# EnricoMiccoli/nodal

Measured on AMD Instinct MI355X. Metric: circuits_per_sec, higher is better.
Workload: dtype f64; 1 GPU; cfg3: grid(1000) 1e6 nodes, sparse CSR path; n=999999, nnz=4995995, parallelism=one GPU

## Files before the change

### nodal_amd/csrc/sagg.hip

```cpp
#include <hip/hip_ext.h>

#include <atomic>
#include <type_traits>

#include "group.h"

int grounded_flags(nodal_ctx *h, uint8_t *flags_dev);

namespace {

using grp::TB;
constexpr int PW = 4;
constexpr int ACAP = 64;
constexpr int RCAP = 96;
constexpr int RCAP_SMALL = 512;
constexpr int RCAP_SMALL_ROWS = 16384;
inline int rcap_for(int64_t nc) { return nc <= RCAP_SMALL_ROWS ? RCAP_SMALL : RCAP; }
constexpr int W0_MAX = 32;
constexpr int COARSEST = 64;
constexpr int MAX_LEVELS = 12;
constexpr int MIS_ROUNDS = 6;
constexpr int TAIL_MAX_N = 1024;
constexpr int TAIL_LEVELS = 6;
constexpr int TAIL_LDS_BUDGET = 150 * 1024;
constexpr int APAD = 32;
constexpr int DOT_BLOCKS = 1024;
#ifndef NODAL_SA_OMEGA
#define NODAL_SA_OMEGA 0.85
#endif
constexpr double OMEGA = NODAL_SA_OMEGA;
constexpr double OMEGA_P = 0.70;
constexpr double OMEGA_P_COARSE = 0.85;
using cyc_t = nodal_cyc_t;

inline unsigned grid_for(int64_t n, unsigned cap = 8192) {
    int64_t g = (n + TB - 1) / TB;
    if (g < 1) g = 1;
    if (g >= 64) g = (g + 7) & ~(int64_t)7;
    return (unsigned)(g > cap ? cap : g);
}
inline int64_t pad64(int64_t n) { return (n + 63) & ~(int64_t)63; }

__device__ __forceinline__ unsigned xcd_block() {
    const unsigned g = gridDim.x, b = blockIdx.x;
    return (g & 7u) ? b : (b & 7u) * (g >> 3) + (b >> 3);
}


struct Ell {
    int64_t n = 0, ld = 0;
    int32_t width = 0;
    const int32_t *col = nullptr;
    const int16_t *dcol = nullptr;
    const double *val = nullptr;
    const float *valf = nullptr;
    const int32_t *len = nullptr;
};

enum { ST_MAXLEN = 0, ST_GRADED = 1, ST_BADDIAG = 2, ST_OVERFLOW = 3, ST_NNZ = 4, ST_UNASSIGNED = 5,
       ST_MAXR = 6, ST_NC = 7 ,
       ST_FARCOL = 8 , ST_COUNT = 9 };

struct SLevel {
    int64_t n = 0, ld = 0, nc = 0;
    int32_t width = 0;
    int32_t maxlen = 0;
    int32_t wfix = 0;
    int64_t nnz = 0;
    DevBuf acol, aval, alen, dinv;
    DevBuf adcol;
    bool d16 = false;
    DevBuf agg, pcol, pval;
    DevBuf rcol, rval, rlen;
    int64_t rld = 0;
    DevBuf vec, part, gflag;
    DevBuf avalf, pvalf, rvalf;
    Ell A() const {
        Ell e;
        e.n = n; e.ld = ld; e.width = width;
        e.col = acol.as<int32_t>(); e.val = aval.as<double>(); e.len = alen.as<int32_t>();
        e.valf = avalf.as<float>();
        e.dcol = d16 ? adcol.as<int16_t>() : nullptr;
        return e;
    }
    template <typename T = double> T *v(int which) const { return reinterpret_cast<T *>(vec.as<double>() + (int64_t)which * ld); }
};
enum { V_X = 0, V_R = 1, V_XP = 2, V_RC = 3, V_C1 = 4, V_C2 = 5, V_V1 = 6, V_V2 = 7, V_R2 = 8, V_X1 = 9, V_T = 10,
       V_COUNT = 11 };

struct TailLevelDesc {
    int n, nc, ld, rld, width, nq, lpr;
    const int32_t *acol, *pcol, *rcol, *rlen, *alen;
    const double *aval, *dinv, *pval, *rval;
    int o_aval, o_acol, o_dinv, o_pval, o_pcol, o_rval, o_rcol, o_B, o_X, o_Y, o_R;
};
struct TailDesc {
    int nlev;
    TailLevelDesc lv[TAIL_LEVELS];
    const double *inv;
    int nu;
    int image_bytes;
    int lds_bytes;
    int skip;
    int slots;
    long long *stamps;
};

struct SHierarchy {
    std::vector<SLevel *> pool;
    int nlev = 0;
    int tail = -1;
    bool ready = false;
    bool kcycle = true;
    bool kfrozen = false;
    int kslot = -1, kcount = 0, ksamples = 0;
    int klevels = 1;
    int nu[3] = {2, 1, 2};
    bool dense_coarsest = true;
    DevBuf tail_stamps, tail_image, apcol, apval, aplen, bstat;
    DevBuf mvec;
    hipEvent_t ev_copy = nullptr;
    hipStream_t aux = nullptr;
    hipEvent_t ev_fork = nullptr, ev_join = nullptr, ev_flags = nullptr;
    bool aux_pending = false;
    bool aux_tried = false;
    bool want_flags = false;
    int flags_levels = 0;
    DevBuf stats, coarse_inv, mis_t, mis_m, mis_flag, mis_id, agg1, keys, rstart, cursor, lists;
    TailDesc td;
    uint64_t *host_stats = nullptr;
    bool sym_valid = false;
    uint64_t sym_epoch = 0;
    int64_t sym_n = 0, sym_nnz = 0;
    bool sym_general = false, sym_check = false;
    int32_t sym_floating = 0;
    hipGraph_t it_graph = nullptr;
    hipGraphExec_t it_exec = nullptr;
    uint64_t it_key = 0;
    bool refreshed = false;
    int last_iters = 0;
    int hint_iters = 0;
    int64_t hint_n = 0, hint_nnz = 0;
    int mblock_iters = 0;
    int64_t mblock_n = 0;
    unsigned long long sym_stats[MAX_LEVELS * ST_COUNT] = {0};
    SLevel *level(int l) {
        while ((int)pool.size() <= l) pool.push_back(new SLevel());
        return pool[l];
    }
    void drop_graph() {
        if (it_exec) (void)hipGraphExecDestroy(it_exec);
        if (it_graph) (void)hipGraphDestroy(it_graph);
        it_exec = nullptr;
        it_graph = nullptr;
        it_key = 0;
    }
    ~SHierarchy() {
        drop_graph();
        if (ev_copy) (void)hipEventDestroy(ev_copy);
        if (ev_fork) (void)hipEventDestroy(ev_fork);
        if (ev_join) (void)hipEventDestroy(ev_join);
        if (ev_flags) (void)hipEventDestroy(ev_flags);
        if (aux) (void)hipStreamDestroy(aux);
        for (SLevel *l : pool) {
            DevBuf *b[] = {&l->acol, &l->aval, &l->alen, &l->dinv, &l->agg, &l->pcol, &l->pval, &l->rcol,
                           &l->rval, &l->rlen, &l->vec, &l->part, &l->gflag, &l->avalf, &l->pvalf, &l->rvalf, &l->adcol};
            for (DevBuf *x : b) x->release();
            delete l;
        }
        tail_image.release();
        mvec.release();
        tail_stamps.release();
        bstat.release();
        apcol.release();
        apval.release();
        aplen.release();
        DevBuf *b[] = {&stats, &coarse_inv, &mis_t, &mis_m, &mis_flag, &mis_id, &agg1, &keys, &rstart, &cursor, &lists};
        for (DevBuf *x : b) x->release();
        if (host_stats) (void)hipHostFree(host_stats);
    }
};


constexpr int BSTAT_MAX = 65536;
__global__ __launch_bounds__(1024) void reduce_bstat(int nblocks, const uint32_t *__restrict__ bstat,
                                                     unsigned long long *__restrict__ stats, int slot_max,
                                                     int slot_sum) {
    __shared__ unsigned int s_max;
    __shared__ unsigned long long s_sum;
    if (threadIdx.x == 0) { s_max = 0; s_sum = 0; }
    __syncthreads();
    unsigned int m = 0;
    unsigned long long t = 0;
    for (int i = threadIdx.x; i < nblocks; i += 1024) {
        m = max(m, bstat[i]);
        t += bstat[BSTAT_MAX + i];
    }
    atomicMax(&s_max, m);
    atomicAdd(&s_sum, t);
    __syncthreads();
    if (threadIdx.x == 0) {
        if (slot_max >= 0) stats[slot_max] = s_max;
        if (slot_sum >= 0) stats[slot_sum] = s_sum;
    }
}

__global__ __launch_bounds__(TB) void row_stats(int64_t n, const int32_t *__restrict__ indptr,
                                                const int32_t *__restrict__ indices,
                                                const double *__restrict__ data, double share, double spread,
                                                bool general, unsigned long long *__restrict__ stats,
                                                uint32_t *__restrict__ bstat) {
    int32_t mlen = 0;
    uint32_t graded = 0, bad = 0, far = 0;
    for (int64_t i = (int64_t)xcd_block() * TB + threadIdx.x; i < n; i += (int64_t)gridDim.x * TB) {
        const int32_t e0 = indptr[i], e1 = indptr[i + 1];
        mlen = max(mlen, e1 - e0);
        double d = 0.0, mx = 0.0, mn = 1e300;
        for (int32_t e = e0; e < e1; ++e) {
            const double v = data[e];
            const int64_t dc = (int64_t)indices[e] - i;
            if (dc > 32767 || dc < -32767) far = 1;
            if (indices[e] == (int32_t)i) d = v;
            else if (v != 0.0) {
                mx = fmax(mx, fabs(v));
                mn = fmin(mn, fabs(v));
                if (v > 0.0 && !general) bad = 1;
            }
        }
        if (!(d > 0.0)) bad = 1;
        graded += (d > 0.0 && (mx > share * d || mx > spread * mn)) ? 1u : 0u;
    }
    __shared__ unsigned int s_len, s_graded, s_bad;
    if (threadIdx.x == 0) s_len = s_graded = s_bad = 0;
    __syncthreads();
    atomicMax(&s_len, (unsigned)mlen);
    if (graded) atomicAdd(&s_graded, graded);
    if (bad) atomicOr(&s_bad, 1u);
    if (far) atomicOr(&s_bad, 2u);
    __syncthreads();
    if (threadIdx.x == 0) {
        bstat[blockIdx.x] = s_len;
        bstat[BSTAT_MAX + blockIdx.x] = s_graded;
        if (s_bad & 1u) atomicOr(&stats[ST_BADDIAG], 1ull);
        if (s_bad & 2u) stats[ST_FARCOL] = 1ull;
    }
}

__global__ __launch_bounds__(TB) void csr_to_ell(int64_t n, int64_t ld, const int32_t *__restrict__ indptr,
                                                 const int32_t *__restrict__ indices,
                                                 const double *__restrict__ data, int32_t *__restrict__ col,
                                                 double *__restrict__ val, float *__restrict__ valf,
                                                 int32_t *__restrict__ len, double *__restrict__ dinv, int32_t wpad,
                                                 int16_t *__restrict__ dcol) {
    for (int64_t i = (int64_t)xcd_block() * TB + threadIdx.x; i < n; i += (int64_t)gridDim.x * TB) {
        const int32_t e0 = indptr[i], e1 = indptr[i + 1];
        double d = 1.0;
        for (int32_t e = e0; e < e1; ++e) {
            const int32_t c = indices[e];
            const double v = data[e];
            col[(int64_t)(e - e0) * ld + i] = c;
            if (dcol) dcol[(int64_t)(e - e0) * ld + i] = (int16_t)(c - (int32_t)i);
            val[(int64_t)(e - e0) * ld + i] = v;
            valf[(int64_t)(e - e0) * ld + i] = (float)v;
            if (c == (int32_t)i) d = v;
        }
        for (int32_t s = e1 - e0; s < wpad; ++s) {
            col[(int64_t)s * ld + i] = (int32_t)i;
            if (dcol) dcol[(int64_t)s * ld + i] = 0;
            val[(int64_t)s * ld + i] = 0.0;
            valf[(int64_t)s * ld + i] = 0.0f;
        }
        len[i] = e1 - e0;
        dinv[i] = 1.0 / d;
    }
}


__device__ __forceinline__ uint32_t hash30(uint32_t x) {
    x ^= x >> 16;
    x *= 0x7feb352du;
    x ^= x >> 15;
    x *= 0x846ca68bu;
    x ^= x >> 16;
    return x & 0x3fffffffu;
}

__global__ __launch_bounds__(TB) void mis_init(int64_t n, uint32_t *__restrict__ T) {
    for (int64_t i = (int64_t)xcd_block() * TB + threadIdx.x; i < n; i += (int64_t)gridDim.x * TB)
        T[i] = (1u << 30) | hash30((uint32_t)i);
}

template <int NB>
__device__ __forceinline__ uint32_t nbr_max_batch(const Ell &A, const uint32_t *__restrict__ v, int64_t i, int32_t l, int32_t s0,
                                                  uint32_t best) {
    int32_t c[NB];
#pragma unroll
    for (int u = 0; u < NB; ++u) c[u] = A.col[(int64_t)(s0 + u < l ? s0 + u : 0) * A.ld + i];
    uint32_t t[NB];
#pragma unroll
    for (int u = 0; u < NB; ++u) t[u] = v[c[u]];
#pragma unroll
    for (int u = 0; u < NB; ++u) best = t[u] > best ? t[u] : best;
    return best;
}
__device__ __forceinline__ uint32_t nbr_max(const Ell &A, const uint32_t *__restrict__ v, int64_t i, int32_t l, uint32_t best) {
    if (l <= 5) return nbr_max_batch<5>(A, v, i, l, 0, best);
    for (int32_t s0 = 0; s0 < l; s0 += 8) best = nbr_max_batch<8>(A, v, i, l, s0, best);
    return best;
}

__global__ __launch_bounds__(TB) void mis_max(Ell A, const uint32_t *__restrict__ v, uint32_t *__restrict__ m) {
    for (int64_t i = (int64_t)xcd_block() * TB + threadIdx.x; i < A.n; i += (int64_t)gridDim.x * TB)
        m[i] = nbr_max(A, v, i, A.len[i], v[i]);
}

__global__ __launch_bounds__(TB) void mis_update(Ell A, uint32_t *__restrict__ T, const uint32_t *__restrict__ m1) {
    for (int64_t i = (int64_t)xcd_block() * TB + threadIdx.x; i < A.n; i += (int64_t)gridDim.x * TB) {
        const uint32_t own = T[i];
        if ((own >> 30) != 1) continue;
        const uint32_t best = nbr_max(A, m1, i, A.len[i], m1[i]);
        if (best == own) T[i] = own | (2u << 30);
        else if ((best >> 30) == 3) T[i] = 0;
    }
}

__global__ __launch_bounds__(TB) void mis_count(int64_t n, const uint32_t *__restrict__ T,
                                                unsigned long long *__restrict__ out) {
    uint32_t left = 0;
    for (int64_t i = (int64_t)xcd_block() * TB + threadIdx.x; i < n; i += (int64_t)gridDim.x * TB)
        left += (T[i] >> 30) == 1 ? 1u : 0u;
#pragma unroll
    for (int off = 32; off > 0; off >>= 1) left += __shfl_down(left, off, 64);
    if ((threadIdx.x & 63) == 0 && left) atomicAdd(out, (unsigned long long)left);
}

__global__ __launch_bounds__(TB) void mis_flag_roots(Ell A, const uint32_t *__restrict__ T,
                                                     uint32_t *__restrict__ flag) {
    for (int64_t i = (int64_t)xcd_block() * TB + threadIdx.x; i <= A.n; i += (int64_t)gridDim.x * TB) {
        uint32_t f = 0;
        if (i < A.n) {
            const uint32_t own = T[i];
            if ((own >> 30) == 3) f = 1;
            else if ((own >> 30) == 1) {
                bool near = false;
                const int32_t l = A.len[i];
                for (int32_t s = 0; s < l; ++s) near = near || (T[A.col[(int64_t)s * A.ld + i]] >> 30) == 3;
                f = near ? 0u : 1u;
            }
        }
        flag[i] = f;
    }
}

constexpr int64_t MIS_SMALL_MAX = 1024;
__global__ __launch_bounds__(1024) void mis_small(Ell A, uint32_t *__restrict__ T, uint32_t *__restrict__ M,
                                                  uint32_t *__restrict__ flag, int rounds) {
    const int64_t n = A.n;
    for (int64_t i = threadIdx.x; i < n; i += 1024) T[i] = (1u << 30) | hash30((uint32_t)i);
    __syncthreads();
    for (int r = 0; r < rounds; ++r) {
        for (int64_t i = threadIdx.x; i < n; i += 1024) {
            uint32_t best = T[i];
            const int32_t l = A.len[i];
            for (int32_t s = 0; s < l; ++s) {
                const uint32_t t = T[A.col[(int64_t)s * A.ld + i]];
                best = t > best ? t : best;
            }
            M[i] = best;
        }
        __syncthreads();
        for (int64_t i = threadIdx.x; i < n; i += 1024) {
            const uint32_t own = T[i];
            if ((own >> 30) != 1) continue;
            uint32_t best = M[i];
            const int32_t l = A.len[i];
            for (int32_t s = 0; s < l; ++s) {
                const uint32_t t = M[A.col[(int64_t)s * A.ld + i]];
                best = t > best ? t : best;
            }
            if (best == own) T[i] = own | (2u << 30);
            else if ((best >> 30) == 3) T[i] = 0;
        }
        __syncthreads();
    }
    for (int64_t i = threadIdx.x; i <= n; i += 1024) {
        uint32_t f = 0;
        if (i < n) {
            const uint32_t own = T[i];
            if ((own >> 30) == 3) f = 1;
            else if ((own >> 30) == 1) {
                bool near = false;
                const int32_t l = A.len[i];
                for (int32_t s = 0; s < l; ++s) near = near || (T[A.col[(int64_t)s * A.ld + i]] >> 30) == 3;
                f = near ? 0u : 1u;
            }
        }
        flag[i] = f;
    }
}

__global__ __launch_bounds__(TB) void assign_near(Ell A, const uint32_t *__restrict__ T,
                                                  const uint32_t *__restrict__ flag,
                                                  const uint32_t *__restrict__ id, int32_t *__restrict__ agg1) {
    for (int64_t i = (int64_t)xcd_block() * TB + threadIdx.x; i < A.n; i += (int64_t)gridDim.x * TB) {
        int32_t a = -1;
        if (flag[i]) a = (int32_t)id[i];
        else {
            uint32_t best = 0;
            const int32_t l = A.len[i];
            auto batch = [&](auto NBc, int32_t s0) {
                constexpr int NB = decltype(NBc)::value;
                int32_t c[NB];
#pragma unroll
                for (int u = 0; u < NB; ++u) c[u] = A.col[(int64_t)(s0 + u < l ? s0 + u : 0) * A.ld + i];
                uint32_t fl[NB], tt[NB], idd[NB];
#pragma unroll
                for (int u = 0; u < NB; ++u) {
                    fl[u] = flag[c[u]];
                    tt[u] = T[c[u]];
                    idd[u] = id[c[u]];
                }
#pragma unroll
                for (int u = 0; u < NB; ++u) {
                    if (s0 + u >= l || c[u] == (int32_t)i || !fl[u]) continue;
                    const uint32_t t = tt[u] | (3u << 30);
                    if (t > best) { best = t; a = (int32_t)idd[u]; }
                }
            };
            if (l <= 5) batch(std::integral_constant<int, 5>{}, 0);
            else for (int32_t s0 = 0; s0 < l; s0 += 8) batch(std::integral_constant<int, 8>{}, s0);
        }
        agg1[i] = a;
    }
}

__global__ __launch_bounds__(TB) void assign_far(Ell A, const int32_t *__restrict__ agg1, int32_t *__restrict__ agg,
                                                 unsigned long long *__restrict__ stats) {
    for (int64_t i = (int64_t)xcd_block() * TB + threadIdx.x; i < A.n; i += (int64_t)gridDim.x * TB) {
        int32_t a = agg1[i];
        if (a < 0) {
            double bw = -1.0;
            const int32_t l = A.len[i];
            auto batch = [&](auto NBc, int32_t s0) {
                constexpr int NB = decltype(NBc)::value;
                int32_t c[NB];
                double w[NB];
#pragma unroll
                for (int u = 0; u < NB; ++u) {
                    const int64_t at = (int64_t)(s0 + u < l ? s0 + u : 0) * A.ld + i;
                    c[u] = A.col[at];
                    w[u] = fabs(A.val[at]);
                }
                int32_t aj[NB];
#pragma unroll
                for (int u = 0; u < NB; ++u) aj[u] = agg1[c[u]];
#pragma unroll
                for (int u = 0; u < NB; ++u) {
                    if (s0 + u >= l || c[u] == (int32_t)i || aj[u] < 0) continue;
                    if (w[u] > bw) { bw = w[u]; a = aj[u]; }
                }
            };
            if (l <= 5) batch(std::integral_constant<int, 5>{}, 0);
            else for (int32_t s0 = 0; s0 < l; s0 += 8) batch(std::integral_constant<int, 8>{}, s0);
            if (a < 0) stats[ST_UNASSIGNED] = 1;
        }
        agg[i] = a;
    }
}

__global__ __launch_bounds__(TB) void build_P(Ell A, const double *__restrict__ dinv,
                                              const int32_t *__restrict__ agg, int32_t *__restrict__ pcol,
                                              double *__restrict__ pval, float *__restrict__ pvalf, double omega_p) {
    for (int64_t i = (int64_t)xcd_block() * TB + threadIdx.x; i < A.n; i += (int64_t)gridDim.x * TB) {
        int32_t c[PW];
        double v[PW];
#pragma unroll
        for (int k = 0; k < PW; ++k) { c[k] = -1; v[k] = 0.0; }
        const int32_t own = agg[i];
        c[0] = own;
        v[0] = 1.0;
        const double wd = omega_p * dinv[i];
        const int32_t l = A.len[i];
        for (int32_t s = 0; s < l; ++s) {
            const int32_t J = agg[A.col[(int64_t)s * A.ld + i]];
            const double t = -wd * A.val[(int64_t)s * A.ld + i];
            bool placed = false;
#pragma unroll
            for (int k = 0; k < PW; ++k) {
                if (!placed && c[k] == J) { v[k] += t; placed = true; }
            }
#pragma unroll
            for (int k = 1; k < PW; ++k) {
                if (!placed && c[k] < 0) { c[k] = J; v[k] = t; placed = true; }
            }
            if (!placed) v[0] += t;
        }
#pragma unroll
        for (int k = 0; k < PW; ++k) {
            pcol[(int64_t)k * A.ld + i] = c[k];
            pval[(int64_t)k * A.ld + i] = v[k];
            pvalf[(int64_t)k * A.ld + i] = (float)v[k];
        }
    }
}

__global__ __launch_bounds__(TB) void r_count(int64_t n, int64_t ld, const int32_t *__restrict__ pcol,
                                              uint32_t *__restrict__ cnt, uint32_t *__restrict__ place) {
    for (int64_t i = (int64_t)xcd_block() * TB + threadIdx.x; i < n; i += (int64_t)gridDim.x * TB) {
#pragma unroll
        for (int k = 0; k < PW; ++k) {
            const int32_t J = pcol[(int64_t)k * ld + i];
            if (J >= 0) place[(int64_t)k * ld + i] = atomicAdd(&cnt[J], 1u);
        }
    }
}
__global__ __launch_bounds__(TB) void r_fill(int64_t n, int64_t ld, const int32_t *__restrict__ pcol,
                                             const uint32_t *__restrict__ rstart, const uint32_t *__restrict__ place,
                                             uint64_t *__restrict__ keys) {
    for (int64_t i = (int64_t)xcd_block() * TB + threadIdx.x; i < n; i += (int64_t)gridDim.x * TB) {
#pragma unroll
        for (int k = 0; k < PW; ++k) {
            const int32_t J = pcol[(int64_t)k * ld + i];
            if (J >= 0) keys[rstart[J] + place[(int64_t)k * ld + i]] = ((uint64_t)i << 2) | (uint64_t)k;
        }
    }
}
__global__ __launch_bounds__(TB) void r_to_ell(int64_t nc, int64_t rld, const uint32_t *__restrict__ rstart,
                                               const uint64_t *__restrict__ keys, int64_t ld,
                                               const double *__restrict__ pval, int32_t *__restrict__ rcol,
                                               double *__restrict__ rval, float *__restrict__ rvalf,
                                               int32_t *__restrict__ rlen,
                                               unsigned long long *__restrict__ stats, uint32_t *__restrict__ bstat,
                                               uint32_t rcap) {
    uint32_t mlen = 0;
    const int sub = threadIdx.x & 7;
    const int64_t rows_per_pass = (int64_t)gridDim.x * (TB / 8);
    for (int64_t I = (int64_t)xcd_block() * (TB / 8) + threadIdx.x / 8; I < nc; I += rows_per_pass) {
        const uint32_t s0 = rstart[I];
        uint32_t l = rstart[I + 1] - s0;
        mlen = l > mlen ? l : mlen;
        if (l > rcap) l = rcap;
        const uint32_t upto = nc <= 4096 ? rcap : ((l + 7u) & ~7u);
        for (uint32_t t = sub; t < upto; t += 8) {
            const int64_t at = ((int64_t)(t >> 3) * rld + I) * 8 + (t & 7);
            if (t < l) {
                const uint64_t key = keys[s0 + t];
                const int64_t i = (int64_t)(key >> 2);
                const double v = pval[(int64_t)(key & 3) * ld + i];
                rcol[at] = (int32_t)i;
                rval[at] = v;
                rvalf[at] = (float)v;
            } else {
                rcol[at] = 0;
                rval[at] = 0.0;
                rvalf[at] = 0.0f;
            }
        }
        if (sub == 0) rlen[I] = (int32_t)l;
    }
    if (mlen > rcap) atomicOr(&stats[ST_OVERFLOW], 2ull);
    __shared__ unsigned int s_max;
    if (threadIdx.x == 0) s_max = 0;
    __syncthreads();
#pragma unroll
    for (int off = 32; off > 0; off >>= 1) {
        const uint32_t o = __shfl_down(mlen, off, 64);
        mlen = o > mlen ? o : mlen;
    }
    if ((threadIdx.x & 63) == 0) atomicMax(&s_max, mlen);
    __syncthreads();
    if (threadIdx.x == 0) {
        bstat[blockIdx.x] = s_max;
        bstat[BSTAT_MAX + blockIdx.x] = 0;
    }
}

__global__ __launch_bounds__(TB) void r_refresh(int64_t nc, int64_t rld, const int32_t *__restrict__ rlen,
                                                const int32_t *__restrict__ rcol, int64_t ld,
                                                const int32_t *__restrict__ pcol, const double *__restrict__ pval,
                                                double *__restrict__ rval, float *__restrict__ rvalf) {
    const int sub = threadIdx.x & 7;
    const int64_t rows_per_pass = (int64_t)gridDim.x * (TB / 8);
    for (int64_t I = (int64_t)xcd_block() * (TB / 8) + threadIdx.x / 8; I < nc; I += rows_per_pass) {
        const int32_t l = rlen[I];
        for (int32_t t = sub; t < l; t += 8) {
            const int64_t at = ((int64_t)(t >> 3) * rld + I) * 8 + (t & 7);
            const int64_t i = rcol[at];
            double v = 0.0;
#pragma unroll
            for (int k = 0; k < PW; ++k) {
                const double pv = pval[(int64_t)k * ld + i];
                v = pcol[(int64_t)k * ld + i] == (int32_t)I ? pv : v;
            }
            rval[at] = v;
            rvalf[at] = (float)v;
        }
    }
}

__global__ __launch_bounds__(TB) void r_sort_short(const uint32_t *__restrict__ rstart, uint64_t *__restrict__ keys,
                                                   int64_t nc) {
    for (int64_t I = (int64_t)xcd_block() * TB + threadIdx.x; I < nc; I += (int64_t)gridDim.x * TB) {
        const uint32_t s0 = rstart[I];
        const int len = (int)(rstart[I + 1] - s0);
        if (len < 2) continue;
        if (len <= 4) grp::sort_short_row<4>(keys + s0, len);
        else if (len <= 8) grp::sort_short_row<8>(keys + s0, len);
        else if (len <= 16) grp::sort_short_row<16>(keys + s0, len);
        else if (len <= 32) grp::sort_short_row<32>(keys + s0, len);
    }
}
__global__ __launch_bounds__(64) void r_sort_medium(const uint32_t *__restrict__ rstart, uint64_t *__restrict__ keys,
                                                    int64_t nc) {
    __shared__ uint64_t buf[RCAP_SMALL];
    const int lane = threadIdx.x;
    for (int64_t I = blockIdx.x; I < nc; I += gridDim.x) {
        const uint32_t s0 = rstart[I];
        const int len = (int)(rstart[I + 1] - s0);
        if (len <= 32 || len > RCAP_SMALL) continue;
        const int P = len <= 64 ? 64 : (len <= 128 ? 128 : (len <= 256 ? 256 : 512));
        for (int e = lane; e < P; e += 64) buf[e] = e < len ? keys[s0 + e] : ~0ull;
        __syncthreads();
        for (int size = 2; size <= P; size <<= 1)
            for (int stride = size >> 1; stride > 0; stride >>= 1) {
                for (int p = lane; p < P / 2; p += 64) {
                    const int i = ((p & ~(stride - 1)) << 1) | (p & (stride - 1));
                    const int j = i | stride;
                    const bool up = (i & size) == 0;
                    const uint64_t a = buf[i], b = buf[j];
                    if ((a > b) == up) { buf[i] = b; buf[j] = a; }
                }
                __syncthreads();
            }
        for (int e = lane; e < len; e += 64) keys[s0 + e] = buf[e];
        __syncthreads();
    }
}

__device__ __forceinline__ int wave_excl_scan(int v, int *total) {
    const int lane = threadIdx.x & 63;
    int incl = v;
#pragma unroll
    for (int off = 1; off < 64; off <<= 1) {
        const int t = __shfl_up(incl, off, 64);
        if (lane >= off) incl += t;
    }
    *total = __shfl(incl, 63, 64);
    return incl - v;
}

template <int APW>
__global__ __launch_bounds__(TB) void ap_rows(Ell A, const int32_t *__restrict__ pcol, const double *__restrict__ pval,
                                              int32_t *__restrict__ apcol, double *__restrict__ apval,
                                              int32_t *__restrict__ aplen, unsigned long long *__restrict__ stats) {
    bool overflow = false;
    for (int64_t i = (int64_t)xcd_block() * TB + threadIdx.x; i < A.n; i += (int64_t)gridDim.x * TB) {
        int32_t c[APW];
        double v[APW];
#pragma unroll
        for (int q = 0; q < APW; ++q) { c[q] = -1; v[q] = 0.0; }
        int cnt = 0;
        const int32_t l = A.len[i];
        for (int32_t s = 0; s < l; ++s) {
            const int32_t k = A.col[(int64_t)s * A.ld + i];
            const double a = A.val[(int64_t)s * A.ld + i];
            int32_t J[PW];
            double pp[PW];
#pragma unroll
            for (int sp = 0; sp < PW; ++sp) {
                J[sp] = pcol[(int64_t)sp * A.ld + k];
                pp[sp] = pval[(int64_t)sp * A.ld + k];
            }
#pragma unroll
            for (int sp = 0; sp < PW; ++sp) {
                if (J[sp] < 0) continue;
                const double t = a * pp[sp];
                bool placed = false;
#pragma unroll
                for (int q = 0; q < APW; ++q)
                    if (!placed && c[q] == J[sp]) { v[q] += t; placed = true; }
#pragma unroll
                for (int q = 0; q < APW; ++q)
                    if (!placed && c[q] < 0) { c[q] = J[sp]; v[q] = t; placed = true; cnt = q + 1; }
                if (!placed) overflow = true;
            }
        }
#pragma unroll
        for (int q = 0; q < APW; ++q)
            if (q < cnt) {
                apcol[(int64_t)q * A.ld + i] = c[q];
                apval[(int64_t)q * A.ld + i] = v[q];
            }
        aplen[i] = cnt;
    }
    if (overflow) atomicOr(&stats[ST_OVERFLOW], 4ull);
}

template <int APW>
__global__ __launch_bounds__(64) void ap_rows_lds(Ell A, const int32_t *__restrict__ pcol,
                                                  const double *__restrict__ pval, int32_t *__restrict__ apcol,
                                                  double *__restrict__ apval, int32_t *__restrict__ aplen,
                                                  unsigned long long *__restrict__ stats) {
    __shared__ int32_t tc[APW * 64];
    __shared__ double tv[APW * 64];
    const int lane = threadIdx.x;
    bool overflow = false;
    for (int64_t i0 = (int64_t)xcd_block() * 64; i0 < A.n; i0 += (int64_t)gridDim.x * 64) {
        const int64_t i = i0 + lane;
#pragma unroll 8
        for (int q = 0; q < APW; ++q) tc[q * 64 + lane] = -1;
        int cnt = 0;
        if (i < A.n) {
            const int32_t l = A.len[i];
            constexpr int AB = 4;
            for (int32_t s0 = 0; s0 < l; s0 += AB) {
                int32_t kk[AB];
                double aa[AB];
#pragma unroll
                for (int u = 0; u < AB; ++u) {
                    const int32_t su = s0 + u < l ? s0 + u : 0;
                    kk[u] = A.col[(int64_t)su * A.ld + i];
                    aa[u] = A.val[(int64_t)su * A.ld + i];
                }
                int32_t J[AB][PW];
                double pp[AB][PW];
#pragma unroll
                for (int u = 0; u < AB; ++u)
#pragma unroll
                    for (int sp = 0; sp < PW; ++sp) {
                        J[u][sp] = pcol[(int64_t)sp * A.ld + kk[u]];
                        pp[u][sp] = pval[(int64_t)sp * A.ld + kk[u]];
                    }
#pragma unroll
                for (int u = 0; u < AB; ++u) {
                    if (s0 + u >= l) continue;
#pragma unroll
                    for (int sp = 0; sp < PW; ++sp) {
                        if (J[u][sp] < 0) continue;
                        const double t = aa[u] * pp[u][sp];
                        uint32_t slot = ((uint32_t)J[u][sp] * 2654435761u) >> 16 & (APW - 1);
                        bool placed = false;
                        for (int probe = 0; probe < APW && !placed; ++probe) {
                            const int32_t c = tc[slot * 64 + lane];
                            if (c == J[u][sp]) {
                                tv[slot * 64 + lane] += t;
                                placed = true;
                            } else if (c < 0) {
                                tc[slot * 64 + lane] = J[u][sp];
                                tv[slot * 64 + lane] = t;
                                ++cnt;
                                placed = true;
                            }
                            slot = (slot + 1) & (APW - 1);
                        }
                        if (!placed) overflow = true;
                    }
                }
            }
            int o = 0;
            for (int q = 0; q < APW; ++q) {
                const int32_t c = tc[q * 64 + lane];
                if (c >= 0) {
                    apcol[(int64_t)o * A.ld + i] = c;
                    apval[(int64_t)o * A.ld + i] = tv[q * 64 + lane];
                    ++o;
                }
            }
            aplen[i] = cnt;
        }
    }
    if (overflow) atomicOr(&stats[ST_OVERFLOW], 4ull);
}

__device__ __forceinline__ int galerkin_products(int64_t ld, const int32_t *__restrict__ apcol,
                                                 const double *__restrict__ apval, const int32_t *__restrict__ aplen,
                                                 int64_t rld, const int32_t *__restrict__ rcol,
                                                 const double *__restrict__ rval, int64_t I, int t0, int tn,
                                                 int32_t *lJ, double *lV) {
    const int lane = threadIdx.x;
    int32_t i = 0, len = 0;
    double w = 0.0;
    if (lane < tn) {
        const int t = t0 + lane;
        const int64_t rat = ((int64_t)(t >> 3) * rld + I) * 8 + (t & 7);
        i = rcol[rat];
        w = rval[rat];
        len = aplen[i];
    }
    int np = 0;
    int o = wave_excl_scan(len, &np);
    constexpr int INFL = 8;
    for (int32_t s0 = 0; s0 < len; s0 += INFL) {
        int32_t cj[INFL];
        double cv[INFL];
#pragma unroll
        for (int q = 0; q < INFL; ++q) {
            const int32_t s = s0 + q < len ? s0 + q : s0;
            cj[q] = apcol[(int64_t)s * ld + i];
            cv[q] = apval[(int64_t)s * ld + i];
        }
#pragma unroll
        for (int q = 0; q < INFL; ++q)
            if (s0 + q < len) {
                lJ[o] = cj[q];
                lV[o] = w * cv[q];
                ++o;
            }
    }
    for (int p = lane + np; p < np + 72; p += 64) lJ[p] = -1;
    __syncthreads();
    return np;
}

template <bool NUMERIC>
__global__ __launch_bounds__(64) void galerkin(int64_t ld, const int32_t *__restrict__ apcol,
                                               const double *__restrict__ apval, const int32_t *__restrict__ aplen,
                                               int64_t nc, int64_t rld, const int32_t *__restrict__ rcol,
                                               const double *__restrict__ rval, const int32_t *__restrict__ rlen,
                                               int64_t cld, int32_t *__restrict__ ccol, double *__restrict__ cval,
                                               float *__restrict__ cvalf,
                                               int32_t *__restrict__ clen, double *__restrict__ cdinv,
                                               unsigned long long *__restrict__ stats, uint32_t *__restrict__ bstat,
                                               int G, int pcap, int maxseg) {
    extern __shared__ __attribute__((aligned(16))) char gsm[];
    int32_t *set = reinterpret_cast<int32_t *>(gsm);
    double *lV = reinterpret_cast<double *>(gsm + 1024);
    int32_t *lJ = reinterpret_cast<int32_t *>(lV + pcap);
    const int lane = threadIdx.x;
    uint32_t my_max = 0, my_nnz = 0, my_flags = 0;
    for (int64_t I = blockIdx.x; I < nc; I += gridDim.x) {
        const int rl = rlen[I];
        const int ngroups = (rl + G - 1) / G;
        int np = 0;
        int total = 0;
        int32_t myJ = 0x7fffffff;
        if constexpr (NUMERIC) {
            total = clen[I];
            if (lane < total) myJ = ccol[(int64_t)lane * cld + I];
        } else {
        for (int k = lane; k < 256; k += 64) set[k] = -1;
        __syncthreads();
        for (int g = 0; g < ngroups; ++g) {
            np = galerkin_products(ld, apcol, apval, aplen, rld, rcol, rval, I, g * G, min(G, rl - g * G), lJ, lV);
            for (int p = lane; p < np; p += 64) {
                const int32_t J = lJ[p];
                uint32_t hsh = ((uint32_t)J * 2654435761u) >> 24;
                for (int probe = 0; probe < 256; ++probe) {
                    const int32_t old = atomicCAS(&set[hsh], -1, J);
                    if (old == -1 || old == J) break;
                    hsh = (hsh + 1) & 255u;
                    if (probe == 255) my_flags |= 1u;
                }
            }
            __syncthreads();
        }
        int32_t mine[4];
        int cnt = 0;
#pragma unroll
        for (int q = 0; q < 4; ++q) {
            mine[q] = set[lane * 4 + q];
            cnt += mine[q] >= 0 ? 1 : 0;
        }
        int off = wave_excl_scan(cnt, &total);
        __syncthreads();
#pragma unroll
        for (int q = 0; q < 4; ++q)
            if (mine[q] >= 0) set[off++] = mine[q];
        __syncthreads();
        if (total > ACAP) {
            my_flags |= 1u;
            total = ACAP;
        }
        myJ = lane < total ? set[lane] : 0x7fffffff;
        __syncthreads();
#pragma unroll
        for (int k = 2; k <= 64; k <<= 1) {
#pragma unroll
            for (int j = k >> 1; j > 0; j >>= 1) {
                const int32_t other = __shfl_xor(myJ, j, 64);
                const bool up = (lane & k) == 0, lower = (lane & j) == 0;
                const int32_t lo = myJ < other ? myJ : other, hi = myJ < other ? other : myJ;
                myJ = (lower == up) ? lo : hi;
            }
        }
        }
        const int nseg = min(maxseg, total <= 16 ? 4 : (total <= 32 ? 2 : 1)), segw = 64 / nseg;
        const int seg = lane / segw;
        const int32_t segJ = __shfl(myJ, lane % segw, 64);
        double acc = 0.0;
        for (int g = 0; g < ngroups; ++g) {
            if (ngroups > 1 || NUMERIC)
                np = galerkin_products(ld, apcol, apval, aplen, rld, rcol, rval, I, g * G, min(G, rl - g * G), lJ, lV);
            int chunk = (((np + nseg - 1) / nseg) + 7) & ~7;
            if (nseg > 1 && ((chunk >> 3) & 1) == 0) chunk += 8;
            for (int p = seg * chunk; p < (seg + 1) * chunk; p += 8) {
                int32_t j8[8];
                double v8[8];
#pragma unroll
                for (int u = 0; u < 8; ++u) {
                    j8[u] = lJ[p + u];
                    v8[u] = lV[p + u];
                }
#pragma unroll
                for (int u = 0; u < 8; ++u) acc += j8[u] == segJ ? v8[u] : 0.0;
            }
            __syncthreads();
        }
        if (nseg == 4) {
            const double a1 = __shfl(acc, lane + 16, 64), a2 = __shfl(acc, lane + 32, 64), a3 = __shfl(acc, lane + 48, 64);
            acc = (acc + a1) + (a2 + a3);
        } else if (nseg == 2) {
            acc += __shfl(acc, lane + 32, 64);
        }
        if (lane >= total && lane < APAD) {
            ccol[(int64_t)lane * cld + I] = (int32_t)I;
            cval[(int64_t)lane * cld + I] = 0.0;
            cvalf[(int64_t)lane * cld + I] = 0.0f;
        }
        if (lane < total) {
            ccol[(int64_t)lane * cld + I] = myJ;
            cval[(int64_t)lane * cld + I] = acc;
            cvalf[(int64_t)lane * cld + I] = (float)acc;
            if (myJ == (int32_t)I) {
                if (!(acc > 0.0)) my_flags |= 4u;
                cdinv[I] = acc > 0.0 ? 1.0 / acc : 1.0;
            }
        }
        if (lane == 0) {
            clen[I] = total;
            my_max = (uint32_t)total > my_max ? (uint32_t)total : my_max;
            my_nnz += (uint32_t)total;
        }
        __syncthreads();
    }
    if (lane == 0) {
        bstat[blockIdx.x] = my_max;
        bstat[BSTAT_MAX + blockIdx.x] = my_nnz;
    }
    if (my_flags & 1u) atomicOr(&stats[ST_OVERFLOW], 1ull);
    if (my_flags & 4u) atomicOr(&stats[ST_BADDIAG], 1ull);
}

__global__ __launch_bounds__(256) void coarsest_inverse(Ell A, double *__restrict__ inv,
                                                        unsigned long long *__restrict__ stats) {
    __shared__ double M[COARSEST][2 * COARSEST + 1];
    const int n = (int)A.n;
    for (int t = threadIdx.x; t < n * 2 * n; t += 256) {
        const int r = t / (2 * n), c = t % (2 * n);
        M[r][c] = (c >= n && c - n == r) ? 1.0 : 0.0;
    }
    __syncthreads();
    for (int r = threadIdx.x; r < n; r += 256)
        for (int s = 0; s < A.len[r]; ++s) M[r][A.col[(int64_t)s * A.ld + r]] = A.val[(int64_t)s * A.ld + r];
    __syncthreads();
    for (int k = 0; k < n; ++k) {
        const double pv = M[k][k];
        if (!(pv > 0.0)) {
            if (threadIdx.x == 0) atomicOr(&stats[ST_BADDIAG], 2ull);
            return;
        }
        const double rp = 1.0 / pv;
        __syncthreads();
        for (int c = threadIdx.x; c < 2 * n; c += 256) M[k][c] *= rp;
        __syncthreads();
        for (int t = threadIdx.x; t < n * 2 * n; t += 256) {
            const int r = t / (2 * n), c = t % (2 * n);
            if (r != k && c != k) M[r][c] = fma(-M[r][k], M[k][c], M[r][c]);
        }
        __syncthreads();
        for (int r = threadIdx.x; r < n; r += 256)
            if (r != k) M[r][k] = 0.0;
        __syncthreads();
    }
    for (int t = threadIdx.x; t < n * n; t += 256) inv[t] = M[t / n][n + t % n];
}

__global__ __launch_bounds__(TB) void flags_up(int64_t n, const int32_t *__restrict__ agg,
                                               const uint8_t *__restrict__ fine, uint8_t *__restrict__ coarse) {
    for (int64_t i = (int64_t)xcd_block() * TB + threadIdx.x; i < n; i += (int64_t)gridDim.x * TB)
        if (fine[i]) coarse[agg[i]] = 1;
}
__global__ __launch_bounds__(64) void last_level_floating(Ell A, const uint8_t *__restrict__ grounded,
                                                          uint32_t *__restrict__ floating) {
    __shared__ int label[COARSEST];
    __shared__ int changed;
    const int n = (int)A.n, i = threadIdx.x;
    if (i < n) label[i] = i;
    __syncthreads();
    for (int it = 0; it < COARSEST; ++it) {
        if (i == 0) changed = 0;
        __syncthreads();
        int best = i < n ? label[i] : 0;
        if (i < n)
            for (int s = 0; s < A.len[i]; ++s) {
                const int l = label[A.col[(int64_t)s * A.ld + i]];
                best = l < best ? l : best;
            }
        __syncthreads();
        if (i < n && best < label[i]) {
            label[i] = best;
            changed = 1;
        }
        __syncthreads();
        if (!changed) break;
        __syncthreads();
    }
    __shared__ int ok[COARSEST];
    if (i < n) ok[i] = 0;
    __syncthreads();
    if (i < n && grounded[i]) ok[label[i]] = 1;
    __syncthreads();
    if (i < n && label[i] == i && !ok[i]) *floating = 1;
}

__global__ __launch_bounds__(TB) void any_unflagged(int64_t n, const uint8_t *__restrict__ grounded,
                                                    uint32_t *__restrict__ floating) {
    for (int64_t i = (int64_t)xcd_block() * TB + threadIdx.x; i < n; i += (int64_t)gridDim.x * TB)
        if (!grounded[i]) *floating = 1;
}

}

#include "sagg_cycle.h"

namespace {

constexpr int SAGG_DECLINED = -3;

int width_class(int maxlen) {
    static const int classes[] = {4, 5, 6, 8, 12, 16, 20, 24, 32};
    for (int c : classes)
        if (maxlen <= c) return c;
    return 0;
}
int choose_wfix(int maxlen, int64_t n, int64_t nnz, int pad_limit) {
    const int c = width_class(maxlen);
    if (c == 0 || c > pad_limit) return 0;
    static const double slack = getenv("NODAL_SA_PADSLACK") ? atof(getenv("NODAL_SA_PADSLACK")) : 1.3;
    if ((double)c * (double)n <= slack * (double)nnz || n <= 32768) return c;
    return 0;
}

SHierarchy *hierarchy_of(nodal_ctx *h) {
    if (!h->sagg) h->sagg = new SHierarchy();
    return static_cast<SHierarchy *>(h->sagg);
}

struct SolveBufs {
    double *r, *p, *p2, *Ap, *part_rz, *part_zap, *part_rr, *part_pap, *sc;
    cyc_t *z, *x0;
    int g0;
};

template <bool NUMERIC>
int galerkin_product(nodal_ctx *h, SHierarchy *H, int l, hipEvent_t r_ready = nullptr, int phase = 0) {
    hipStream_t st = h->stream;
    SLevel *L = H->level(l), *C = H->level(l + 1);
    const int64_t n = L->n, ld = L->ld, nc = C->n;
    Ell A = L->A();
    A.width = L->maxlen;
    unsigned long long *dstats = H->stats.as<unsigned long long>();
    const int apw = A.width <= 6 ? 16 : 64;
    NODAL_HIP_TRY(h, H->apcol.reserve((size_t)apw * ld * 4 + 64));
    NODAL_HIP_TRY(h, H->apval.reserve((size_t)apw * ld * 8 + 64));
    NODAL_HIP_TRY(h, H->aplen.reserve((size_t)ld * 4 + 64));
    int32_t *apcol = H->apcol.as<int32_t>(), *aplen = H->aplen.as<int32_t>();
    double *apval = H->apval.as<double>();
    unsigned long long *lst = dstats + (size_t)l * ST_COUNT;
    const unsigned g = grid_for(n);
    if (phase != 2) {
        switch (apw) {
        case 16: ap_rows<16><<<g, TB, 0, st>>>(A, L->pcol.as<int32_t>(), L->pval.as<double>(), apcol, apval, aplen, lst); break;
        default: {
            const unsigned gl = (unsigned)((n + 63) / 64 < 4096 ? (n + 63) / 64 : 4096);
            ap_rows_lds<64><<<gl, 64, 0, st>>>(A, L->pcol.as<int32_t>(), L->pval.as<double>(), apcol, apval, aplen, lst);
        } break;
        }
        NODAL_HIP_TRY(h, hipGetLastError());
    }
    if (phase == 1) return NODAL_OK;
    int G = 1024 / apw;
    G = (G < 8 ? 8 : (G > 64 ? 64 : G));
    static const int g_env = getenv("NODAL_SA_GG") ? atoi(getenv("NODAL_SA_GG")) : 40;
    if (g_env >= 8 && g_env <= 64 && apw == 16) G = g_env & ~7;
    const int pcap = G * apw + 72;
    const size_t lds = 1024 + (size_t)pcap * 12;
    static const int64_t gcap = getenv("NODAL_SA_GCAP") ? atoll(getenv("NODAL_SA_GCAP")) : 16384;
    static const int maxseg = getenv("NODAL_SA_GSEG") ? atoi(getenv("NODAL_SA_GSEG")) : 4;
    const unsigned gg = (unsigned)(nc < gcap ? nc : (gcap < BSTAT_MAX ? gcap : BSTAT_MAX));
    if (r_ready) NODAL_HIP_TRY(h, hipStreamWaitEvent(st, r_ready, 0));
    galerkin<NUMERIC><<<gg, 64, lds, st>>>(
        ld, apcol, apval, aplen, nc, L->rld, L->rcol.as<int32_t>(), L->rval.as<double>(), L->rlen.as<int32_t>(),
        C->ld, C->acol.as<int32_t>(), C->aval.as<double>(), C->avalf.as<float>(), C->alen.as<int32_t>(),
        C->dinv.as<double>(), dstats + (size_t)(l + 1) * ST_COUNT, H->bstat.as<uint32_t>(), G, pcap, maxseg);
    if (!NUMERIC)
        reduce_bstat<<<1, 1024, 0, st>>>((int)gg, H->bstat.as<uint32_t>(), dstats + (size_t)(l + 1) * ST_COUNT,
                                         ST_MAXLEN, ST_NNZ);
    NODAL_HIP_TRY(h, hipGetLastError());
    return NODAL_OK;
}

double omega_p(int level) {
    static double w[2] = {-1.0, -1.0};
    if (w[0] < 0.0) {
        double a = OMEGA_P, b = OMEGA_P_COARSE;
        if (const char *e = getenv("NODAL_SA_OMEGA_P")) {
            a = atof(e);
            const char *c = strchr(e, ',');
            b = c ? atof(c + 1) : a;
        }
        w[1] = b > 0.0 && b < 1.2 ? b : OMEGA_P_COARSE;
        w[0] = a > 0.0 && a < 1.0 ? a : OMEGA_P;
    }
    return w[level > 0 ? 1 : 0];
}

int build_level(nodal_ctx *h, SHierarchy *H, int l, unsigned long long *hs, bool *declined, bool *stop) {
    hipStream_t st = h->stream;
    SLevel *L = H->level(l);
    const int64_t n = L->n, ld = L->ld;
    Ell A = L->A();
    A.width = L->maxlen;
    unsigned long long *dstats = H->stats.as<unsigned long long>();

    NODAL_HIP_TRY(h, H->mis_t.reserve((size_t)n * 8 + 64));
    NODAL_HIP_TRY(h, H->mis_m.reserve((size_t)n * 8 + 64));
    NODAL_HIP_TRY(h, H->mis_flag.reserve((size_t)(n + 1) * 4 + 64));
    NODAL_HIP_TRY(h, H->mis_id.reserve((size_t)(n + 1) * 4 + 64 + scan_tmp_bytes(n + 1)));
    NODAL_HIP_TRY(h, H->agg1.reserve((size_t)n * 4 + 64));
    NODAL_HIP_TRY(h, L->agg.reserve((size_t)n * 4 + 64));
    NODAL_HIP_TRY(h, H->cursor.reserve((MIS_ROUNDS + 2) * 8 + 64));
    uint32_t *T = H->mis_t.as<uint32_t>(), *M = H->mis_m.as<uint32_t>();
    uint32_t *flag = H->mis_flag.as<uint32_t>(), *id = H->mis_id.as<uint32_t>();
    unsigned long long *cnt = H->cursor.as<unsigned long long>();
    void *scan_tmp = H->mis_id.as<char>() + (((size_t)(n + 1) * 4 + 63) & ~(size_t)63);

    const unsigned g = grid_for(n);
    static const bool trace_mis = getenv("NODAL_TRACE") != nullptr;
    if (trace_mis) NODAL_HIP_TRY(h, hipMemsetAsync(cnt, 0, (MIS_ROUNDS + 2) * 8, st));
    static const int mis_rounds = getenv("NODAL_SA_MIS") ? std::min(MIS_ROUNDS, std::max(1, atoi(getenv("NODAL_SA_MIS")))) : MIS_ROUNDS;
    if (n <= MIS_SMALL_MAX && !trace_mis) {
        mis_small<<<1, 1024, 0, st>>>(A, T, M, flag, mis_rounds);
    } else {
        mis_init<<<g, TB, 0, st>>>(n, T);
        for (int r = 0; r < mis_rounds; ++r) {
            mis_max<<<g, TB, 0, st>>>(A, T, M);
            mis_update<<<g, TB, 0, st>>>(A, T, M);
            if (trace_mis) mis_count<<<g, TB, 0, st>>>(n, T, cnt + r + 1);
        }
        mis_flag_roots<<<grid_for(n + 1), TB, 0, st>>>(A, T, flag);
    }
    NODAL_HIP_TRY(h, hipGetLastError());
    NODAL_TRY(scan_exclusive_u32(h, flag, id, n + 1, reinterpret_cast<uint32_t *>(dstats + (size_t)l * ST_COUNT + ST_NC),
                                 scan_tmp));
    NODAL_HIP_TRY(h, hipMemcpyAsync(hs, dstats, (size_t)MAX_LEVELS * ST_COUNT * 8, hipMemcpyDeviceToHost, st));
    unsigned long long hcnt[MIS_ROUNDS + 1] = {0};
    if (trace_mis) NODAL_HIP_TRY(h, hipMemcpyAsync(hcnt, cnt, sizeof hcnt, hipMemcpyDeviceToHost, st));
    if (!H->ev_copy) NODAL_HIP_TRY(h, hipEventCreateWithFlags(&H->ev_copy, hipEventDisableTiming));
    NODAL_HIP_TRY(h, hipEventRecord(H->ev_copy, st));
    NODAL_HIP_TRY(h, L->pcol.reserve((size_t)PW * ld * 4 + 64));
    NODAL_HIP_TRY(h, L->pval.reserve((size_t)PW * ld * 8 + 64));
    NODAL_HIP_TRY(h, L->pvalf.reserve((size_t)PW * ld * 4 + 64));
    assign_near<<<g, TB, 0, st>>>(A, T, flag, id, H->agg1.as<int32_t>());
    assign_far<<<g, TB, 0, st>>>(A, H->agg1.as<int32_t>(), L->agg.as<int32_t>(), dstats + (size_t)l * ST_COUNT);
    build_P<<<g, TB, 0, st>>>(A, L->dinv.as<double>(), L->agg.as<int32_t>(), L->pcol.as<int32_t>(),
                             L->pval.as<double>(), L->pvalf.as<float>(), omega_p(l));
    NODAL_HIP_TRY(h, hipGetLastError());
    NODAL_WAIT_EVENT(h, H->ev_copy, st);
    if (trace_mis) {
        fprintf(stderr, "[sagg] level %d: undecided after each MIS round:", l);
        for (int r = 1; r <= MIS_ROUNDS; ++r) fprintf(stderr, " %llu", hcnt[r]);
        fprintf(stderr, "\n");
    }
    const int64_t nc = (int64_t)(hs[(size_t)l * ST_COUNT + ST_NC] & 0xffffffffull);
    if (l > 0) {
        const unsigned long long *s = hs + (size_t)l * ST_COUNT;
        L->maxlen = (int32_t)s[ST_MAXLEN];
        L->nnz = (int64_t)s[ST_NNZ];
        A.width = L->maxlen;
        if (s[ST_OVERFLOW] || s[ST_BADDIAG] || hs[(size_t)(l - 1) * ST_COUNT + ST_OVERFLOW] ||
            hs[(size_t)(l - 1) * ST_COUNT + ST_UNASSIGNED]) {
            *declined = true;
            return NODAL_OK;
        }
    }
    if (nc >= n || L->maxlen <= 1) {
        *stop = true;
        return NODAL_OK;
    }
    if ((nc * 2 > n && n > 4096) || nc < 1) {
        *declined = true;
        return NODAL_OK;
    }
    L->nc = nc;

    static const bool fork_allowed = !(getenv("NODAL_SA_FORK") && atoi(getenv("NODAL_SA_FORK")) == 0);
    if (H->aux && !nodal_extra_streams_ok(h) && nodal_calls_in_flight() <= 1) {
        NODAL_WAIT_STREAM(h, H->aux);
        (void)hipStreamDestroy(H->aux);
        H->aux = nullptr;
        H->aux_tried = false;
    }
    if (fork_allowed && !H->aux_tried && nodal_extra_streams_ok(h)) {
        H->aux_tried = true;
        if (hipStreamCreateWithFlags(&H->aux, hipStreamNonBlocking) != hipSuccess) H->aux = nullptr;
        if (H->aux && ((!H->ev_fork && hipEventCreateWithFlags(&H->ev_fork, hipEventDisableTiming) != hipSuccess) ||
                       (!H->ev_join && hipEventCreateWithFlags(&H->ev_join, hipEventDisableTiming) != hipSuccess) ||
                       (!H->ev_flags && hipEventCreateWithFlags(&H->ev_flags, hipEventDisableTiming) != hipSuccess))) {
            (void)hipStreamDestroy(H->aux);
            H->aux = nullptr;
        }
        (void)hipGetLastError();
    }
    const bool forked = fork_allowed && H->aux != nullptr && nodal_extra_streams_ok(h);
    const size_t a4 = (((size_t)(nc + 1) * 4) + 255) & ~(size_t)255;
    const size_t scan2 = (scan_tmp_bytes(nc + 1) + 255) & ~(size_t)255;
    NODAL_HIP_TRY(h, H->rstart.reserve(a4 + 256 + scan2 + (size_t)PW * ld * 4 + 64));
    NODAL_HIP_TRY(h, H->keys.reserve((size_t)PW * n * 8 + 64));
    SLevel *C = H->level(l + 1);
    C->n = nc;
    C->ld = pad64(nc);
    C->width = ACAP;
    C->nc = 0;
    L->rld = C->ld;
    const int rcap = rcap_for(nc);
    NODAL_HIP_TRY(h, L->rcol.reserve((size_t)rcap * C->ld * 4 + 64));
    NODAL_HIP_TRY(h, L->rval.reserve((size_t)rcap * C->ld * 8 + 64));
    NODAL_HIP_TRY(h, L->rvalf.reserve((size_t)rcap * C->ld * 4 + 64));
    NODAL_HIP_TRY(h, L->rlen.reserve((size_t)C->ld * 4 + 64));
    NODAL_HIP_TRY(h, C->acol.reserve((size_t)ACAP * C->ld * 4 + 64));
    NODAL_HIP_TRY(h, C->aval.reserve((size_t)ACAP * C->ld * 8 + 64));
    NODAL_HIP_TRY(h, C->avalf.reserve((size_t)ACAP * C->ld * 4 + 64));
    NODAL_HIP_TRY(h, C->alen.reserve((size_t)C->ld * 4 + 64));
    NODAL_HIP_TRY(h, C->dinv.reserve((size_t)C->ld * 8 + 64));
    if (forked && H->want_flags) {
        if (l == 0) NODAL_HIP_TRY(h, L->gflag.reserve((size_t)n + 64));
        NODAL_HIP_TRY(h, C->gflag.reserve((size_t)C->n + 64));
    }
    {
        const int apw = L->maxlen <= 6 ? 16 : 64;
        NODAL_HIP_TRY(h, H->apcol.reserve((size_t)apw * ld * 4 + 64));
        NODAL_HIP_TRY(h, H->apval.reserve((size_t)apw * ld * 8 + 64));
        NODAL_HIP_TRY(h, H->aplen.reserve((size_t)ld * 4 + 64));
    }
    hipStream_t main_st = h->stream;
    struct StreamGuard {
        nodal_ctx *h;
        hipStream_t keep;
        ~StreamGuard() { h->stream = keep; }
    } guard{h, main_st};
    if (forked) {
        NODAL_HIP_TRY(h, hipEventRecord(H->ev_fork, main_st));
        NODAL_HIP_TRY(h, hipStreamWaitEvent(H->aux, H->ev_fork, 0));
        H->aux_pending = true;
        NODAL_TRY(galerkin_product<false>(h, H, l, nullptr, 1));
        h->stream = H->aux;
        st = H->aux;
    }
    char *rs = H->rstart.as<char>();
    uint32_t *rstart = reinterpret_cast<uint32_t *>(rs);
    void *scan_tmp2 = rs + a4 + 256;
    uint32_t *place = reinterpret_cast<uint32_t *>(rs + a4 + 256 + scan2);
    NODAL_HIP_TRY(h, hipMemsetAsync(rs, 0, a4 + 256, st));
    r_count<<<g, TB, 0, st>>>(n, ld, L->pcol.as<int32_t>(), rstart, place);
    NODAL_HIP_TRY(h, hipGetLastError());
    NODAL_TRY(scan_exclusive_u32(h, rstart, rstart, nc + 1, nullptr, scan_tmp2));
    uint64_t *keys = H->keys.as<uint64_t>();
    r_fill<<<g, TB, 0, st>>>(n, ld, L->pcol.as<int32_t>(), rstart, place, keys);
    r_sort_short<<<grid_for(nc), TB, 0, st>>>(rstart, keys, nc);
    r_sort_medium<<<(unsigned)(nc < 8192 ? nc : 8192), 64, 0, st>>>(rstart, keys, nc);
    NODAL_HIP_TRY(h, hipGetLastError());

    {
        const unsigned gr = grid_for(nc * 8);
        r_to_ell<<<gr, TB, 0, st>>>(nc, L->rld, rstart, keys, ld, L->pval.as<double>(), L->rcol.as<int32_t>(),
                                   L->rval.as<double>(), L->rvalf.as<float>(), L->rlen.as<int32_t>(),
                                   dstats + (size_t)l * ST_COUNT, H->bstat.as<uint32_t>(), (uint32_t)rcap);
        reduce_bstat<<<1, 1024, 0, st>>>((int)gr, H->bstat.as<uint32_t>(), dstats + (size_t)l * ST_COUNT, ST_MAXR, -1);
    }
    if (forked) {
        NODAL_HIP_TRY(h, hipGetLastError());
        NODAL_HIP_TRY(h, hipEventRecord(H->ev_join, H->aux));
        if (H->want_flags && H->flags_levels == l) {
            if (l == 0) NODAL_TRY(grounded_flags(h, L->gflag.as<uint8_t>()));
            NODAL_HIP_TRY(h, hipMemsetAsync(C->gflag.p, 0, ((size_t)C->n + 63) & ~(size_t)63, st));
            flags_up<<<grid_for(n), TB, 0, st>>>(n, L->agg.as<int32_t>(), L->gflag.as<uint8_t>(), C->gflag.as<uint8_t>());
            NODAL_HIP_TRY(h, hipGetLastError());
            NODAL_HIP_TRY(h, hipEventRecord(H->ev_flags, H->aux));
            H->flags_levels = l + 1;
        }
        h->stream = main_st;
        st = main_st;
    }
    NODAL_TRY(galerkin_product<false>(h, H, l, forked ? H->ev_join : nullptr, forked ? 2 : 0));
    if (forked && H->flags_levels != l + 1) H->aux_pending = false;
    return NODAL_OK;
}

const void *tail_kernel(int slots) {
    return slots <= 8 ? reinterpret_cast<const void *>(k_tail<8>)
                      : slots <= 16 ? reinterpret_cast<const void *>(k_tail<16>)
                                    : reinterpret_cast<const void *>(k_tail<32>);
}

int build_tail(nodal_ctx *h, SHierarchy *H, const unsigned long long *hs) {
    H->tail = -1;
    const int last = H->nlev - 1;
    auto up16 = [](int x) { return (x + 15) & ~15; };
    for (int t = 1; t <= last; ++t) {
        if (H->pool[t]->n > TAIL_MAX_N || last - t + 1 > TAIL_LEVELS) continue;
        TailDesc d;
        memset(&d, 0, sizeof d);
        d.nlev = last - t + 1;
        d.nu = getenv("NODAL_SA_TAIL_NU") ? atoi(getenv("NODAL_SA_TAIL_NU")) : 3;
        if (d.nu < 1) d.nu = 1;
        int off = 0;
        for (int k = 0; k < d.nlev; ++k) {
            const SLevel *L = H->pool[t + k];
            TailLevelDesc &q = d.lv[k];
            q.n = (int)L->n; q.nc = (int)L->nc; q.ld = (int)L->ld; q.rld = (int)L->rld; q.width = L->maxlen;
            q.acol = L->acol.as<int32_t>(); q.aval = L->aval.as<double>();
            q.dinv = L->dinv.as<double>(); q.alen = L->alen.as<int32_t>();
            q.pcol = L->pcol.as<int32_t>(); q.pval = L->pval.as<double>();
            q.rcol = L->rcol.as<int32_t>(); q.rval = L->rval.as<double>(); q.rlen = L->rlen.as<int32_t>();
            if (k == d.nlev - 1) {
                q.o_aval = off; off = up16(off + (H->dense_coarsest ? q.n * q.n : q.n) * 8);
                continue;
            }
            const int maxr = (int)hs[(size_t)(t + k) * ST_COUNT + ST_MAXR];
            q.nq = (maxr + 7) / 8;
            q.lpr = 1;
            while (q.lpr < 8 && q.n * q.lpr * 2 <= 1024) q.lpr *= 2;
            q.o_aval = off; off = up16(off + q.n * q.width * 8);
            q.o_acol = off; off = up16(off + q.n * q.width * 2);
            q.o_dinv = off; off = up16(off + q.n * 8);
            q.o_pval = off; off = up16(off + q.n * PW * 8);
            q.o_pcol = off; off = up16(off + q.n * PW * 2);
            q.o_rval = off; off = up16(off + q.nq * q.nc * 8 * 8);
            q.o_rcol = off; off = up16(off + q.nq * q.nc * 8 * 2);
        }
        d.image_bytes = off;
        for (int k = 0; k < d.nlev; ++k) {
            TailLevelDesc &q = d.lv[k];
            q.o_B = off; off = up16(off + q.n * 8);
            q.o_X = off; off = up16(off + q.n * 8);
            if (k == d.nlev - 1) continue;
            q.o_Y = off; off = up16(off + q.n * 8);
            q.o_R = off; off = up16(off + q.n * 8);
        }
        d.inv = H->dense_coarsest ? H->coarse_inv.as<double>() : nullptr;
        d.skip = d.nlev > 1 ? d.lv[0].o_dinv : 0;
        d.lds_bytes = off - d.skip;
        if (getenv("NODAL_TAIL_PROBE")) {
            NODAL_HIP_TRY(h, H->tail_stamps.reserve(64 * sizeof(long long)));
            d.stamps = H->tail_stamps.as<long long>();
        }
        if (d.lds_bytes > TAIL_LDS_BUDGET) continue;
        d.slots = d.nlev > 1 ? (d.lv[0].width + d.lv[0].lpr - 1) / d.lv[0].lpr : 1;
        if (d.slots > 32) continue;
        {
            static std::atomic<bool> lds_allowed[64][3];
            const int dev = h->device >= 0 && h->device < 64 ? h->device : 0;
            const int which = d.slots <= 8 ? 0 : (d.slots <= 16 ? 1 : 2);
            if (!lds_allowed[dev][which].load(std::memory_order_acquire)) {
                NODAL_HIP_TRY(h, hipFuncSetAttribute(tail_kernel(d.slots), hipFuncAttributeMaxDynamicSharedMemorySize,
                                                     TAIL_LDS_BUDGET));
                lds_allowed[dev][which].store(true, std::memory_order_release);
            }
        }
        NODAL_HIP_TRY(h, H->tail_image.reserve((size_t)d.image_bytes + 256));
        k_tail_pack<<<1, 1024, 0, h->stream>>>(d, H->tail_image.as<char>());
        NODAL_HIP_TRY(h, hipGetLastError());
        H->td = d;
        H->tail = t;
        break;
    }
    return NODAL_OK;
}

int sagg_refresh(nodal_ctx *h, SHierarchy *H, const int32_t *indptr0, const int32_t *indices0, const double *data0,
                 bool general, bool *ok) {
    *ok = false;
    hipStream_t st = h->stream;
    unsigned long long *dstats = H->stats.as<unsigned long long>();
    unsigned long long *hs = reinterpret_cast<unsigned long long *>(H->host_stats);
    NODAL_HIP_TRY(h, hipMemsetAsync(dstats, 0, (size_t)MAX_LEVELS * ST_COUNT * 8, st));
    SLevel *L0 = H->pool[0];
    const int64_t n0 = L0->n;
    {
        const unsigned gr = grid_for(n0);
        static const double spread = getenv("NODAL_SA_SPREAD") ? atof(getenv("NODAL_SA_SPREAD")) : 16.0;
        static const double share = getenv("NODAL_SA_SHARE") ? atof(getenv("NODAL_SA_SHARE")) : 0.9;
        row_stats<<<gr, TB, 0, st>>>(n0, indptr0, indices0, data0, share, spread, general, dstats, H->bstat.as<uint32_t>());
        reduce_bstat<<<1, 1024, 0, st>>>((int)gr, H->bstat.as<uint32_t>(), dstats, ST_MAXLEN, ST_GRADED);
    }
    csr_to_ell<<<grid_for(n0), TB, 0, st>>>(n0, L0->ld, indptr0, indices0, data0, L0->acol.as<int32_t>(),
                                           L0->aval.as<double>(), L0->avalf.as<float>(),
                                           L0->alen.as<int32_t>(), L0->dinv.as<double>(), L0->wfix,
                                           L0->d16 ? L0->adcol.as<int16_t>() : nullptr);
    NODAL_HIP_TRY(h, hipGetLastError());
    for (int l = 0; l + 1 < H->nlev; ++l) {
        SLevel *L = H->pool[l], *C = H->pool[l + 1];
        Ell A = L->A();
        A.width = L->maxlen;
        build_P<<<grid_for(L->n), TB, 0, st>>>(A, L->dinv.as<double>(), L->agg.as<int32_t>(), L->pcol.as<int32_t>(),
                                              L->pval.as<double>(), L->pvalf.as<float>(), omega_p(l));
        const bool forked = H->aux != nullptr && nodal_extra_streams_ok(h) &&
                            !(getenv("NODAL_SA_FORK") && atoi(getenv("NODAL_SA_FORK")) == 0);
        hipStream_t rst = st;
        if (forked) {
            NODAL_HIP_TRY(h, hipEventRecord(H->ev_fork, st));
            NODAL_HIP_TRY(h, hipStreamWaitEvent(H->aux, H->ev_fork, 0));
            H->aux_pending = true;
            NODAL_TRY(galerkin_product<true>(h, H, l, nullptr, 1));
            rst = H->aux;
        }
        r_refresh<<<grid_for(C->n * 8), TB, 0, rst>>>(C->n, L->rld, L->rlen.as<int32_t>(), L->rcol.as<int32_t>(), L->ld,
                                                     L->pcol.as<int32_t>(), L->pval.as<double>(), L->rval.as<double>(),
                                                     L->rvalf.as<float>());
        NODAL_HIP_TRY(h, hipGetLastError());
        if (forked) NODAL_HIP_TRY(h, hipEventRecord(H->ev_join, H->aux));
        NODAL_TRY(galerkin_product<true>(h, H, l, forked ? H->ev_join : nullptr, forked ? 2 : 0));
        if (forked) H->aux_pending = false;
    }
    const int last = H->nlev - 1;
    if (H->dense_coarsest)
        coarsest_inverse<<<1, 256, 0, st>>>(H->pool[last]->A(), H->coarse_inv.as<double>(), dstats + (size_t)last * ST_COUNT);
    if (H->tail >= 0) k_tail_pack<<<1, 1024, 0, st>>>(H->td, H->tail_image.as<char>());
    NODAL_HIP_TRY(h, hipGetLastError());
    NODAL_HIP_TRY(h, hipMemcpyAsync(hs, dstats, (size_t)MAX_LEVELS * ST_COUNT * 8, hipMemcpyDeviceToHost, st));
    NODAL_WAIT_STREAM(h, st);
    const int64_t bar = n0 / 100 < 32 ? (n0 / 100 > 0 ? n0 / 100 : 1) : 32;
    if (hs[ST_BADDIAG] || (int64_t)hs[ST_GRADED] >= bar) return NODAL_OK;
    for (int k = 1; k < H->nlev; ++k)
        if (hs[(size_t)k * ST_COUNT + ST_BADDIAG] || hs[(size_t)k * ST_COUNT + ST_OVERFLOW]) return NODAL_OK;
    *ok = true;
    return NODAL_OK;
}

}

void sagg_destroy(nodal_ctx *h) {
    delete static_cast<SHierarchy *>(h->sagg);
    h->sagg = nullptr;
}

static int sagg_setup_csr_body(nodal_ctx *h, int64_t n0, int64_t nnz0, const int32_t *indptr0, const int32_t *indices0,
                               const double *data0, bool general, bool check_floating, bool *accepted, int32_t *floating);

int sagg_setup_csr(nodal_ctx *h, int64_t n0, int64_t nnz0, const int32_t *indptr0, const int32_t *indices0,
                   const double *data0, bool general, bool check_floating, bool *accepted, int32_t *floating) {
    const int s = sagg_setup_csr_body(h, n0, nnz0, indptr0, indices0, data0, general, check_floating, accepted, floating);
    SHierarchy *H = static_cast<SHierarchy *>(h->sagg);
    if (H && H->aux && H->aux_pending && H->ev_flags) {
        if (hipEventRecord(H->ev_flags, H->aux) == hipSuccess) (void)hipStreamWaitEvent(h->stream, H->ev_flags, 0);
        H->aux_pending = false;
        (void)hipGetLastError();
    }
    return s;
}

static int sagg_setup_csr_body(nodal_ctx *h, int64_t n0, int64_t nnz0, const int32_t *indptr0, const int32_t *indices0,
                               const double *data0, bool general, bool check_floating, bool *accepted, int32_t *floating) {
    *accepted = false;
    *floating = 0;
    static const bool enabled = !(getenv("NODAL_SAGG") && atoi(getenv("NODAL_SAGG")) == 0);
    static const bool trace = getenv("NODAL_TRACE") != nullptr;
    if (!enabled) return NODAL_OK;
    SHierarchy *H = hierarchy_of(h);
    H->ready = false;
    hipStream_t st = h->stream;
    if (n0 >= (1ll << 30)) return NODAL_OK;
    static const bool reuse = !(getenv("NODAL_SA_REUSE") && atoi(getenv("NODAL_SA_REUSE")) == 0);
    if (reuse && H->sym_valid && H->sym_epoch == h->struct_epoch && H->sym_n == n0 && H->sym_nnz == nnz0 &&
        H->sym_general == general && H->sym_check == check_floating) {
        bool ok = false;
        NODAL_TRY(sagg_refresh(h, H, indptr0, indices0, data0, general, &ok));
        if (ok) {
            *floating = H->sym_floating;
            H->refreshed = true;
            H->ready = true;
            *accepted = true;
            if (trace) fprintf(stderr, "[sagg] symbolic setup kept (struct epoch %llu): values refreshed\n",
                               (unsigned long long)h->struct_epoch);
            return NODAL_OK;
        }
        if (trace) fprintf(stderr, "[sagg] the kept hierarchy does not take the new values: full setup\n");
    }
    H->sym_valid = false;
    H->refreshed = false;
    H->want_flags = check_floating;
    H->flags_levels = 0;
    H->last_iters = 0;
    H->drop_graph();
    NODAL_HIP_TRY(h, H->stats.reserve((size_t)MAX_LEVELS * ST_COUNT * 8 + 64));
    if (!H->host_stats)
        NODAL_HIP_TRY(h, hipHostMalloc(reinterpret_cast<void **>(&H->host_stats), (size_t)MAX_LEVELS * ST_COUNT * 8 + 64));
    unsigned long long *dstats = H->stats.as<unsigned long long>();
    unsigned long long *hs = reinterpret_cast<unsigned long long *>(H->host_stats);
    NODAL_HIP_TRY(h, hipMemsetAsync(dstats, 0, (size_t)MAX_LEVELS * ST_COUNT * 8, st));
    NODAL_HIP_TRY(h, H->bstat.reserve((size_t)2 * BSTAT_MAX * 4 + 64));
    {
        const unsigned gr = grid_for(n0);
        static const double spread = getenv("NODAL_SA_SPREAD") ? atof(getenv("NODAL_SA_SPREAD")) : 16.0;
        static const double share = getenv("NODAL_SA_SHARE") ? atof(getenv("NODAL_SA_SHARE")) : 0.9;
        row_stats<<<gr, TB, 0, st>>>(n0, indptr0, indices0, data0, share, spread, general, dstats, H->bstat.as<uint32_t>());
        reduce_bstat<<<1, 1024, 0, st>>>((int)gr, H->bstat.as<uint32_t>(), dstats, ST_MAXLEN, ST_GRADED);
    }
    NODAL_HIP_TRY(h, hipGetLastError());
    NODAL_HIP_TRY(h, hipMemcpyAsync(hs, dstats, ST_COUNT * 8, hipMemcpyDeviceToHost, st));
    NODAL_WAIT_STREAM(h, st);
    const int64_t bar = n0 / 100 < 32 ? (n0 / 100 > 0 ? n0 / 100 : 1) : 32;
    if (hs[ST_MAXLEN] > (unsigned long long)W0_MAX || hs[ST_MAXLEN] == 0 || hs[ST_BADDIAG] ||
        (int64_t)hs[ST_GRADED] >= bar) {
        if (trace)
            fprintf(stderr, "[sagg] declined: longest row %llu, graded nodes %llu (bar %lld), M-matrix %s\n",
                    hs[ST_MAXLEN], hs[ST_GRADED], (long long)bar, hs[ST_BADDIAG] ? "no" : "yes");
        return NODAL_OK;
    }
    SLevel *L0 = H->level(0);
    L0->n = n0;
    L0->ld = pad64(n0);
    L0->maxlen = (int32_t)hs[ST_MAXLEN];
    L0->nnz = nnz0;
    L0->wfix = choose_wfix(L0->maxlen, n0, nnz0, 8);
    L0->width = L0->wfix ? L0->wfix : L0->maxlen;
    NODAL_HIP_TRY(h, L0->acol.reserve((size_t)L0->width * L0->ld * 4 + 64));
    NODAL_HIP_TRY(h, L0->aval.reserve((size_t)L0->width * L0->ld * 8 + 64));
    NODAL_HIP_TRY(h, L0->avalf.reserve((size_t)L0->width * L0->ld * 4 + 64));
    NODAL_HIP_TRY(h, L0->alen.reserve((size_t)L0->ld * 4 + 64));
    NODAL_HIP_TRY(h, L0->dinv.reserve((size_t)L0->ld * 8 + 64));
    static const bool d16_env = !(getenv("NODAL_SA_D16") && atoi(getenv("NODAL_SA_D16")) == 0);
    L0->d16 = d16_env && hs[ST_FARCOL] == 0;
    if (L0->d16) NODAL_HIP_TRY(h, L0->adcol.reserve((size_t)L0->width * L0->ld * 2 + 64));
    csr_to_ell<<<grid_for(n0), TB, 0, st>>>(n0, L0->ld, indptr0, indices0, data0, L0->acol.as<int32_t>(),
                                           L0->aval.as<double>(), L0->avalf.as<float>(),
                                           L0->alen.as<int32_t>(), L0->dinv.as<double>(), L0->wfix,
                                           L0->d16 ? L0->adcol.as<int16_t>() : nullptr);
    NODAL_HIP_TRY(h, hipGetLastError());

    int l = 0;
    bool diag_last = false;
    for (;; ++l) {
        SLevel *L = H->level(l);
        if (L->n <= COARSEST && l > 0) break;
        if (l + 1 >= MAX_LEVELS) {
            if (trace) fprintf(stderr, "[sagg] declined: more than %d levels\n", MAX_LEVELS);
            return NODAL_OK;
        }
        bool declined = false, stop = false;
        NODAL_TRY(build_level(h, H, l, hs, &declined, &stop));
        if (declined) {
            if (trace)
                fprintf(stderr, "[sagg] declined at level %d (%lld rows): does not coarsen / over a cap / not positive "
                                "(this level: overflow %llx baddiag %llx; level above: overflow %llx unassigned %llu maxr %llu)\n",
                        l, (long long)L->n, hs[(size_t)l * ST_COUNT + ST_OVERFLOW], hs[(size_t)l * ST_COUNT + ST_BADDIAG],
                        l > 0 ? hs[(size_t)(l - 1) * ST_COUNT + ST_OVERFLOW] : 0ull,
                        l > 0 ? hs[(size_t)(l - 1) * ST_COUNT + ST_UNASSIGNED] : 0ull,
                        l > 0 ? hs[(size_t)(l - 1) * ST_COUNT + ST_MAXR] : 0ull);
            return NODAL_OK;
        }
        if (stop) {
            diag_last = true;
            break;
        }
    }
    H->nlev = l + 1;
    SLevel *last = H->level(l);
    if (H->nlev < 2) return NODAL_OK;
    NODAL_HIP_TRY(h, hipMemcpyAsync(hs, dstats, (size_t)MAX_LEVELS * ST_COUNT * 8, hipMemcpyDeviceToHost, st));
    if (!H->ev_copy) NODAL_HIP_TRY(h, hipEventCreateWithFlags(&H->ev_copy, hipEventDisableTiming));
    NODAL_HIP_TRY(h, hipEventRecord(H->ev_copy, st));
    if (check_floating) {
        if (H->flags_levels == 0) {
            NODAL_HIP_TRY(h, H->level(0)->gflag.reserve((size_t)n0 + 64));
            NODAL_TRY(grounded_flags(h, H->level(0)->gflag.as<uint8_t>()));
        } else {
            NODAL_HIP_TRY(h, hipStreamWaitEvent(st, H->ev_flags, 0));
            H->aux_pending = false;
        }
        for (int k = H->flags_levels; k + 1 < H->nlev; ++k) {
            SLevel *L = H->pool[k], *C = H->pool[k + 1];
            NODAL_HIP_TRY(h, C->gflag.reserve((size_t)C->n + 64));
            NODAL_HIP_TRY(h, hipMemsetAsync(C->gflag.p, 0, ((size_t)C->n + 63) & ~(size_t)63, st));
            flags_up<<<grid_for(L->n), TB, 0, st>>>(L->n, L->agg.as<int32_t>(), L->gflag.as<uint8_t>(),
                                                   C->gflag.as<uint8_t>());
        }
        NODAL_HIP_TRY(h, hipGetLastError());
    }
    NODAL_WAIT_EVENT(h, H->ev_copy, st);
    for (int k = 0; k < H->nlev; ++k) {
        const unsigned long long *s = hs + (size_t)k * ST_COUNT;
        if (k > 0) {
            H->pool[k]->maxlen = (int32_t)s[ST_MAXLEN];
            H->pool[k]->nnz = (int64_t)s[ST_NNZ];
            H->pool[k]->wfix = choose_wfix(H->pool[k]->maxlen, H->pool[k]->n, H->pool[k]->nnz, APAD);
        }
        if (s[ST_OVERFLOW] || (k > 0 && s[ST_BADDIAG]) || s[ST_UNASSIGNED]) {
            if (trace) fprintf(stderr, "[sagg] declined: level %d over a cap / not positive\n", k);
            return NODAL_OK;
        }
    }
    diag_last = last->maxlen <= 1;
    H->dense_coarsest = !diag_last;
    if (H->dense_coarsest) {
        if (last->n > COARSEST) return NODAL_OK;
        NODAL_HIP_TRY(h, H->coarse_inv.reserve((size_t)last->n * last->n * 8 + 64));
        coarsest_inverse<<<1, 256, 0, st>>>(last->A(), H->coarse_inv.as<double>(),
                                            dstats + (size_t)l * ST_COUNT);
        NODAL_HIP_TRY(h, hipGetLastError());
    }
    for (int k = 0; k < H->nlev; ++k) {
        SLevel *L = H->pool[k];
        NODAL_HIP_TRY(h, L->vec.reserve((size_t)V_COUNT * L->ld * 8 + 256));
        NODAL_HIP_TRY(h, L->part.reserve(5 * DOT_BLOCKS * 8 + 512));
    }
    NODAL_TRY(build_tail(h, H, hs));

    if (!check_floating) {
        NODAL_HIP_TRY(h, hipMemcpyAsync(hs, dstats, (size_t)MAX_LEVELS * ST_COUNT * 8, hipMemcpyDeviceToHost, st));
        NODAL_WAIT_STREAM(h, st);
        if (hs[(size_t)l * ST_COUNT + ST_BADDIAG] & 2ull) return NODAL_OK;
    } else {
        uint32_t *fl = reinterpret_cast<uint32_t *>(dstats + (size_t)(MAX_LEVELS - 1) * ST_COUNT + ST_COUNT - 1);
        if (H->dense_coarsest) last_level_floating<<<1, 64, 0, st>>>(last->A(), last->gflag.as<uint8_t>(), fl);
        else any_unflagged<<<grid_for(last->n), TB, 0, st>>>(last->n, last->gflag.as<uint8_t>(), fl);
        NODAL_HIP_TRY(h, hipGetLastError());
        NODAL_HIP_TRY(h, hipMemcpyAsync(hs, dstats, (size_t)MAX_LEVELS * ST_COUNT * 8, hipMemcpyDeviceToHost, st));
        NODAL_WAIT_STREAM(h, st);
        if (hs[(size_t)l * ST_COUNT + ST_BADDIAG] & 2ull) {
            if (trace) fprintf(stderr, "[sagg] declined: coarsest matrix not positive definite\n");
            return NODAL_OK;
        }
        *floating = hs[(size_t)(MAX_LEVELS - 1) * ST_COUNT + ST_COUNT - 1] != 0 ? 1 : 0;
    }
    if (trace) {
        fprintf(stderr, "[sagg] levels (rows/entries/longest row/padded width):");
        for (int k = 0; k < H->nlev; ++k)
            fprintf(stderr, " %lld/%lld/%d/%d", (long long)H->pool[k]->n, (long long)H->pool[k]->nnz,
                    H->pool[k]->maxlen, H->pool[k]->wfix);
        fprintf(stderr, "  tail %d (%d register slots)  coarsest %s\n", H->tail, H->tail >= 0 ? H->td.slots : 0,
                H->dense_coarsest ? "dense" : "diagonal");
    }
    H->ready = true;
    *accepted = true;
    H->sym_valid = true;
    H->sym_epoch = h->struct_epoch;
    H->sym_n = n0;
    H->sym_nnz = nnz0;
    H->sym_general = general;
    H->sym_check = check_floating;
    H->sym_floating = *floating;
    memcpy(H->sym_stats, hs, sizeof H->sym_stats);
    return NODAL_OK;
}

int sagg_setup(nodal_ctx *h, bool *accepted, int32_t *floating) {
    return sagg_setup_csr(h, h->n, h->nnz, h->indptr.as<int32_t>(), h->indices.as<int32_t>(), h->data.as<double>(),
                          false, true, accepted, floating);
}

namespace {

int last_level(nodal_ctx *h, SHierarchy *H, int l, const double *b, double *out) {
    hipStream_t st = h->stream;
    SLevel *L = H->pool[l];
    const int64_t n = L->n;
    if (l == H->tail) {
        if (H->td.slots <= 8) k_tail<8><<<1, 1024, (size_t)H->td.lds_bytes, st>>>(H->td, H->tail_image.as<char>(), b, out, 1);
        else if (H->td.slots <= 16) k_tail<16><<<1, 1024, (size_t)H->td.lds_bytes, st>>>(H->td, H->tail_image.as<char>(), b, out, 1);
        else k_tail<32><<<1, 1024, (size_t)H->td.lds_bytes, st>>>(H->td, H->tail_image.as<char>(), b, out, 1);
    } else {
        k_coarsest<<<grid_for(n), TB, 0, st>>>(n, H->dense_coarsest ? H->coarse_inv.as<double>() : nullptr,
                                               L->dinv.as<double>(), b, out);
    }
    NODAL_HIP_TRY(h, hipGetLastError());
    return NODAL_OK;
}

void kcycle_schedule(SHierarchy *H, int it) {
    static const bool on = !(getenv("NODAL_SA_KFREEZE") && atoi(getenv("NODAL_SA_KFREEZE")) == 0);
    H->kfrozen = false;
    H->kslot = -1;
    if (!on || it < 0) return;
    if (it == 0) H->ksamples = 0;
    const bool adaptive = it < 4 || (it & 3) == 0;
    if (!adaptive && H->ksamples > 0) {
        H->kfrozen = true;
    } else if (it >= 2) {
        H->kslot = H->ksamples % 3;
        ++H->ksamples;
        H->kcount = H->ksamples < 3 ? H->ksamples : 3;
    }
}

template <typename TBV, typename TOUT>
int cycle(nodal_ctx *h, SHierarchy *H, int l, const TBV *b, const cyc_t *x0, TOUT *out, const SolveBufs *sb) {
    hipStream_t st = h->stream;
    SLevel *L = H->pool[l];
    const int64_t n = L->n;
    SLevel *C = H->pool[l + 1];
    const int64_t nc = C->n;
    const Ell A = L->A();
    const double *dinv = L->dinv.as<double>();
    const cyc_t *x = x0;
    cyc_t *r = L->v<cyc_t>(V_R), *xp = L->v<cyc_t>(V_XP);
    const unsigned g = sb ? (unsigned)sb->g0 : grid_for(n);
    const unsigned tb = L->wfix ? TB : TB * LPR_RAGGED;
    const int nu = H->nu[l < 2 ? l : 2];
    if (nu >= 2) {
        cyc_t *x1 = L->v<cyc_t>(V_X1);
        SAGG_DISPATCH_W(L->wfix, (k_post<W, false, TBV, cyc_t><<<g, tb, 0, st>>>(A, dinv, b, x0, x1, nullptr, nullptr, nullptr)));
        x = x1;
    }
    if (nu >= 3) {
        cyc_t *x2 = L->v<cyc_t>(V_T);
        SAGG_DISPATCH_W(L->wfix, (k_post<W, false, TBV, cyc_t><<<g, tb, 0, st>>>(A, dinv, b, x, x2, nullptr, nullptr, nullptr)));
        x = x2;
    }
    SAGG_DISPATCH_W(L->wfix, (k_smooth_residual<W, TBV><<<g, tb, 0, st>>>(A, b, x, r)));
    const bool last = l + 1 == H->tail || l + 1 == H->nlev - 1;
    const double *coef = nullptr;
    if (last) {
        double *rc = C->v<double>(V_RC), *c1 = C->v<double>(V_C1);
        k_restrict<double><<<grid_for(nc * RL), TB, 0, st>>>(nc, L->rld, L->rcol.as<int32_t>(), L->rvalf.as<float>(),
                                                            L->rlen.as<int32_t>(), r, rc, C->dinv.as<double>(), nullptr);
        NODAL_HIP_TRY(h, hipGetLastError());
        NODAL_TRY(last_level(h, H, l + 1, rc, c1));
        k_prolong<double><<<grid_for(n), TB, 0, st>>>(n, L->ld, L->pcol.as<int32_t>(), L->pvalf.as<float>(), x, c1,
                                                     (const double *)nullptr, nullptr, xp);
    } else {
        cyc_t *rc = C->v<cyc_t>(V_RC), *c1 = C->v<cyc_t>(V_C1), *c2 = C->v<cyc_t>(V_C2), *x0c = C->v<cyc_t>(V_X);
        k_restrict<cyc_t><<<grid_for(nc * RL), TB, 0, st>>>(nc, L->rld, L->rcol.as<int32_t>(), L->rvalf.as<float>(),
                                                           L->rlen.as<int32_t>(), r, rc, C->dinv.as<double>(), x0c);
        NODAL_HIP_TRY(h, hipGetLastError());
        int nparts = 0;
        const bool kcycle = l < H->klevels && H->kcycle;
        if (kcycle) {
            cyc_t *v1 = C->v<cyc_t>(V_V1), *v2 = C->v<cyc_t>(V_V2), *r2 = C->v<cyc_t>(V_R2);
            double *part = C->part.as<double>();
            const Ell Ac = C->A();
            const unsigned gd = grid_for(nc, DOT_BLOCKS);
            const unsigned tbc = C->wfix ? TB : TB * LPR_RAGGED;
            nparts = (int)gd;
            double *cf = part + 5 * DOT_BLOCKS;
            if (H->kfrozen && l == 0) {
                NODAL_TRY((cycle<cyc_t, cyc_t>(h, H, l + 1, rc, x0c, c1, nullptr)));
                SAGG_DISPATCH_W(C->wfix, (k_spmv_resid<W><<<gd, tbc, 0, st>>>(Ac, c1, rc, cf + 3, r2, C->dinv.as<double>(), x0c)));
                NODAL_HIP_TRY(h, hipGetLastError());
                NODAL_TRY((cycle<cyc_t, cyc_t>(h, H, l + 1, r2, x0c, c2, nullptr)));
                coef = cf + 3;
                nparts = 0;
            } else {
                NODAL_TRY((cycle<cyc_t, cyc_t>(h, H, l + 1, rc, x0c, c1, nullptr)));
                SAGG_DISPATCH_W(C->wfix, (k_spmv_dots<W><<<gd, tbc, 0, st>>>(Ac, c1, v1, rc, nullptr, part + 0 * DOT_BLOCKS,
                                                                            part + 1 * DOT_BLOCKS, nullptr)));
                k_second_residual<<<grid_for(nc), TB, 0, st>>>(nc, rc, v1, part, nparts, r2, C->dinv.as<double>(), x0c);
                NODAL_HIP_TRY(h, hipGetLastError());
                NODAL_TRY((cycle<cyc_t, cyc_t>(h, H, l + 1, r2, x0c, c2, nullptr)));
                SAGG_DISPATCH_W(C->wfix, (k_spmv_dots<W><<<gd, tbc, 0, st>>>(Ac, c2, v2, v1, r2, part + 3 * DOT_BLOCKS,
                                                                            part + 2 * DOT_BLOCKS, part + 4 * DOT_BLOCKS)));
                NODAL_HIP_TRY(h, hipGetLastError());
            }
        } else {
            NODAL_TRY((cycle<cyc_t, cyc_t>(h, H, l + 1, rc, x0c, c1, nullptr)));
        }
        if (nparts) {
            double *cf = C->part.as<double>() + 5 * DOT_BLOCKS;
            const bool sample = l == 0 && H->kslot >= 0;
            k_kcoef<<<1, 320, 0, st>>>(C->part.as<double>(), nparts, cf, sample ? H->kslot : -1, sample ? H->kcount : 0);
            coef = cf;
        }
        k_prolong<cyc_t><<<grid_for(n), TB, 0, st>>>(n, L->ld, L->pcol.as<int32_t>(), L->pvalf.as<float>(), x, c1, c2, coef,
                                                    xp);
    }
    const cyc_t *cur = xp;
    if (nu >= 2) {
        cyc_t *mid = L->v<cyc_t>(V_T);
        SAGG_DISPATCH_W(L->wfix, (k_post<W, false, TBV, cyc_t><<<g, tb, 0, st>>>(A, dinv, b, cur, mid, nullptr, nullptr, nullptr)));
        cur = mid;
    }
    if (nu >= 3) {
        cyc_t *mid2 = L->v<cyc_t>(V_X1);
        SAGG_DISPATCH_W(L->wfix, (k_post<W, false, TBV, cyc_t><<<g, tb, 0, st>>>(A, dinv, b, cur, mid2, nullptr, nullptr, nullptr)));
        cur = mid2;
    }
    if (sb) {
        SAGG_DISPATCH_W(L->wfix, (k_post<W, true, TBV, TOUT><<<g, tb, 0, st>>>(A, dinv, b, cur, out, sb->Ap, sb->part_rz,
                                                                              sb->part_zap)));
    } else {
        SAGG_DISPATCH_W(L->wfix, (k_post<W, false, TBV, TOUT><<<g, tb, 0, st>>>(A, dinv, b, cur, out, nullptr, nullptr, nullptr)));
    }
    NODAL_HIP_TRY(h, hipGetLastError());
    return NODAL_OK;
}

__global__ void f_set_scalars(double *__restrict__ sc, double tol2) {
    for (int k = 0; k < F_COUNT; ++k) sc[k] = 0.0;
    sc[F_TOL2] = tol2;
}

size_t align_up(size_t x) { return (x + 255) & ~(size_t)255; }

}

__global__ __launch_bounds__(TB) void k_x0(int64_t n, const double *__restrict__ dinv, const double *__restrict__ r,
                                           cyc_t *__restrict__ x0) {
    for (int64_t i = (int64_t)xcd_block() * TB + threadIdx.x; i < n; i += (int64_t)gridDim.x * TB)
        x0[i] = (cyc_t)(OMEGA * dinv[i] * r[i]);
}
bool sagg_ready(nodal_ctx *h, int64_t n) {
    SHierarchy *H = static_cast<SHierarchy *>(h->sagg);
    return H && H->ready && H->pool[0]->n == n;
}
void sagg_invalidate(nodal_ctx *h) {
    if (h->sagg) static_cast<SHierarchy *>(h->sagg)->ready = false;
}
int sagg_levels(nodal_ctx *h) { return h->sagg ? static_cast<SHierarchy *>(h->sagg)->nlev : 0; }
bool sagg_x0_slot(nodal_ctx *h, const double **dinv, nodal_cyc_t **x0, int64_t *n0, double *omega) {
    SHierarchy *H = static_cast<SHierarchy *>(h->sagg);
    if (!H || !H->ready) return false;
    SLevel *L0 = H->pool[0];
    *dinv = L0->dinv.as<double>();
    *x0 = L0->v<cyc_t>(V_X);
    *n0 = L0->n;
    *omega = OMEGA;
    return true;
}
int sagg_apply(nodal_ctx *h, const double *r, double *z, bool x0_ready, int it) {
    SHierarchy *H = static_cast<SHierarchy *>(h->sagg);
    if (!H || !H->ready) return nodal_fail(h, NODAL_E_INVALID, "sagg_setup_csr not called");
    SLevel *L0 = H->pool[0];
    cyc_t *x0 = L0->v<cyc_t>(V_X);
    if (!x0_ready) k_x0<<<grid_for(L0->n), TB, 0, h->stream>>>(L0->n, L0->dinv.as<double>(), r, x0);
    NODAL_HIP_TRY(h, hipGetLastError());
    kcycle_schedule(H, it);
    const int rc = cycle<double, double>(h, H, 0, r, x0, z, nullptr);
    H->kfrozen = false;
    H->kslot = -1;
    return rc;
}

int sagg_spmv(nodal_ctx *h, const double *x, double *y, hipEvent_t start, hipEvent_t stop) {
    SHierarchy *H = static_cast<SHierarchy *>(h->sagg);
    if (!H || !H->ready) return nodal_fail(h, NODAL_E_INVALID, "sagg_setup_csr not called");
    const SLevel *L0 = H->pool[0];
    const Ell A0 = L0->A();
    const unsigned tb0 = L0->wfix ? TB : TB * LPR_RAGGED;
    if (start && stop) {
        SAGG_DISPATCH_W(L0->wfix, (hipExtLaunchKernelGGL((k_ell_spmv<W>), dim3(grid_for(L0->n)), dim3(tb0), 0, h->stream,
                                                         start, stop, 0, A0, x, y)));
    } else {
        SAGG_DISPATCH_W(L0->wfix, (k_ell_spmv<W><<<grid_for(L0->n), tb0, 0, h->stream>>>(A0, x, y)));
    }
    NODAL_HIP_TRY(h, hipGetLastError());
    return NODAL_OK;
}

int sagg_fcg_solve(nodal_ctx *h, const double *b, bool do_setup, int32_t *info, int32_t *iters, double *resid) {
    static const bool trace = getenv("NODAL_TRACE") != nullptr;
    const int64_t n = h->n;
    hipStream_t st = h->stream;
    SHierarchy *H = hierarchy_of(h);
    if (do_setup) {
        bool accepted = false;
        int32_t floating = 0;
        NODAL_TRY(sagg_setup(h, &accepted, &floating));
        if (!accepted) return SAGG_DECLINED;
        if (floating) {
            *info = 1;
            *iters = 0;
            *resid = 0.0;
            return -2;
        }
    }
    if (!H->ready || H->pool[0]->n != n) return SAGG_DECLINED;
    h->amg_levels = H->nlev;
    static const int kc = getenv("NODAL_SA_KCYCLE") ? atoi(getenv("NODAL_SA_KCYCLE")) : 1;
    H->kcycle = kc != 0;
    H->klevels = getenv("NODAL_SA_KLEVELS") ? atoi(getenv("NODAL_SA_KLEVELS")) : 1;
    if (const char *e = getenv("NODAL_SA_NU")) {
        for (int k = 0; k < 3 && e[k] >= '1' && e[k] <= '3'; ++k) H->nu[k] = e[k] - '0';
    }

    const size_t vec = align_up((size_t)n * 8);
    NODAL_HIP_TRY(h, h->solver.reserve(6 * vec + 4 * MAX_PARTIALS * 8 + F_COUNT * 8 + 256));
    char *base = h->solver.as<char>();
    SolveBufs sb;
    sb.r = reinterpret_cast<double *>(base);
    sb.z = reinterpret_cast<cyc_t *>(base + vec);
    sb.p = reinterpret_cast<double *>(base + 2 * vec);
    sb.Ap = reinterpret_cast<double *>(base + 3 * vec);
    sb.x0 = reinterpret_cast<cyc_t *>(base + 4 * vec);
    sb.p2 = reinterpret_cast<double *>(base + 5 * vec);
    sb.part_rz = reinterpret_cast<double *>(base + 6 * vec);
    sb.part_zap = sb.part_rz + MAX_PARTIALS;
    sb.part_rr = sb.part_zap + MAX_PARTIALS;
    sb.part_pap = sb.part_rr + MAX_PARTIALS;
    sb.sc = sb.part_pap + MAX_PARTIALS;
    sb.g0 = (int)grid_for(n, MAX_PARTIALS);
    double *x = h->x.as<double>();
    const Ell A0 = H->pool[0]->A();

    const double tol = 1e-13;
    f_set_scalars<<<1, 1, 0, st>>>(sb.sc, tol * tol);
    const double *dinv0 = H->pool[0]->dinv.as<double>();
    f_init<<<sb.g0, TB, 0, st>>>(b, x, sb.r, sb.Ap, dinv0, sb.x0, sb.part_rr, n);
    NODAL_HIP_TRY(h, hipGetLastError());

    const int64_t maxit = getenv("NODAL_FCG_MAXIT") ? atoll(getenv("NODAL_FCG_MAXIT")) : 2000;
    hipEvent_t e0 = h->ev[2], e1 = h->ev[3];
    h->kern_ms = 0;
    h->kern_launches = 0;
    double hs[F_COUNT];
    int64_t enqueued = 0;
    int batch = 6;
    if (H->last_iters > 6 && (H->refreshed || !do_setup)) batch = H->last_iters + 1 > 32 ? 32 : H->last_iters + 1;
    else if (H->hint_iters > 8 && H->hint_n == n && H->hint_nnz == H->pool[0]->nnz) {
        batch = (3 * H->hint_iters) / 4;
        if (batch > 32) batch = 32;
    }
    int status = 0;
    const bool poll_partials = !(getenv("NODAL_FCG_HOST_SUM") && atoi(getenv("NODAL_FCG_HOST_SUM")) == 0);
    double rr_prev = -1.0;
    int64_t it_prev = 0;
    int polls = 0;
    static const bool fuse_dir_env = !(getenv("NODAL_SA_FUSE_DIR") && atoi(getenv("NODAL_SA_FUSE_DIR")) == 0);
    const bool fuse_dir = fuse_dir_env && LPR_RAGGED == 1;
    static const bool graphs_env = getenv("NODAL_SA_GRAPH") && atoi(getenv("NODAL_SA_GRAPH")) != 0;
    auto iteration = [&](int it, bool timed) -> int {
        kcycle_schedule(H, graphs_env ? -1 : it);
        struct KReset {
            SHierarchy *H;
            ~KReset() { H->kfrozen = false; H->kslot = -1; }
        } kreset{H};
        NODAL_TRY((cycle<double, cyc_t>(h, H, 0, sb.r, sb.x0, sb.z, &sb)));
        if (fuse_dir) {
            double *p_new = (it & 1) ? sb.p2 : sb.p;
            const double *p_old = (it & 1) ? sb.p : sb.p2;
            const unsigned tbf = TB;
            if (timed) {
                SAGG_DISPATCH_W(H->pool[0]->wfix, (hipExtLaunchKernelGGL((f_dir_spmv<W>), dim3(sb.g0), dim3(tbf), 0, st, e0, e1, 0,
                                                                         A0, (const cyc_t *)sb.z, p_old, p_new, sb.Ap,
                                                                         (const double *)sb.part_rz, (const double *)sb.part_zap,
                                                                         (const double *)sb.part_rr, sb.g0, sb.part_pap, sb.sc,
                                                                         it & 1)));
            } else {
                SAGG_DISPATCH_W(H->pool[0]->wfix, (f_dir_spmv<W><<<sb.g0, tbf, 0, st>>>(A0, sb.z, p_old, p_new, sb.Ap, sb.part_rz,
                                                                                       sb.part_zap, sb.part_rr, sb.g0,
                                                                                       sb.part_pap, sb.sc, it & 1)));
            }
            f_update<<<sb.g0, TB, 0, st>>>(x, sb.r, p_new, sb.Ap, sb.part_pap, sb.g0, dinv0, sb.x0, sb.part_rr, sb.sc, it & 1, n);
            NODAL_HIP_TRY(h, hipGetLastError());
            return NODAL_OK;
        }
        f_direction<<<sb.g0, TB, 0, st>>>(sb.z, sb.p, sb.part_rz, sb.part_zap, sb.part_rr, sb.g0, sb.sc, it & 1, n);
        const unsigned tb0 = H->pool[0]->wfix ? TB : TB * LPR_RAGGED;
        if (timed) {
            SAGG_DISPATCH_W(H->pool[0]->wfix, (hipExtLaunchKernelGGL((f_spmv<W>), dim3(sb.g0), dim3(tb0), 0, st, e0, e1, 0,
                                                                     A0, (const double *)sb.p, sb.Ap, sb.part_pap,
                                                                     (const double *)sb.sc, it & 1)));
        } else {
            SAGG_DISPATCH_W(H->pool[0]->wfix, (f_spmv<W><<<sb.g0, tb0, 0, st>>>(A0, sb.p, sb.Ap, sb.part_pap, sb.sc, it & 1)));
        }
        f_update<<<sb.g0, TB, 0, st>>>(x, sb.r, sb.p, sb.Ap, sb.part_pap, sb.g0, dinv0, sb.x0, sb.part_rr, sb.sc, it & 1, n);
        NODAL_HIP_TRY(h, hipGetLastError());
        return NODAL_OK;
    };
    static const bool graphs = getenv("NODAL_SA_GRAPH") && atoi(getenv("NODAL_SA_GRAPH")) != 0;
    if (graphs && (H->refreshed || !do_setup)) {
        uint64_t key = 1469598103934665603ull;
        auto mix = [&](uint64_t v) { key = (key ^ v) * 1099511628211ull; };
        mix((uint64_t)(uintptr_t)base); mix((uint64_t)(uintptr_t)x); mix((uint64_t)n); mix((uint64_t)sb.g0);
        mix((uint64_t)H->nlev); mix((uint64_t)(H->tail + 1)); mix((uint64_t)H->kcycle); mix((uint64_t)H->klevels);
        mix((uint64_t)(H->nu[0] * 100 + H->nu[1] * 10 + H->nu[2])); mix((uint64_t)H->td.lds_bytes);
        mix((uint64_t)(uintptr_t)H->tail_image.p); mix((uint64_t)(uintptr_t)H->coarse_inv.p);
        for (int k = 0; k < H->nlev; ++k) {
            const SLevel *L = H->pool[k];
            const void *ps[] = {L->acol.p, L->aval.p, L->avalf.p, L->alen.p, L->dinv.p, L->pcol.p, L->pvalf.p,
                                L->rcol.p, L->rvalf.p, L->rlen.p, L->vec.p, L->part.p};
            for (const void *q : ps) mix((uint64_t)(uintptr_t)q);
            mix((uint64_t)L->n); mix((uint64_t)L->ld); mix((uint64_t)L->wfix); mix((uint64_t)L->rld);
        }
        if (H->it_exec && H->it_key != key) H->drop_graph();
        if (!H->it_exec) {
            hipGraph_t g = nullptr;
            hipGraphExec_t ex = nullptr;
            if (hipStreamBeginCapture(st, hipStreamCaptureModeThreadLocal) == hipSuccess) {
                int cs = iteration(0, false);
                if (cs == NODAL_OK) cs = iteration(1, false);
                const hipError_t ce = hipStreamEndCapture(st, &g);
                if (cs == NODAL_OK && ce == hipSuccess && g && hipGraphInstantiate(&ex, g, nullptr, nullptr, 0) == hipSuccess) {
                    H->it_graph = g;
                    H->it_exec = ex;
                    H->it_key = key;
                } else {
                    if (g) (void)hipGraphDestroy(g);
                    (void)hipGetLastError();
                }
            } else {
                (void)hipGetLastError();
            }
        }
    } else if (H->it_exec && do_setup) {
        H->drop_graph();
    }
    while (status == 0) {
        for (int c = 0; c < batch;) {
            if (H->it_exec && c > 0 && c + 1 < batch && (enqueued & 1) == 0) {
                NODAL_HIP_TRY(h, hipGraphLaunch(H->it_exec, st));
                c += 2;
                enqueued += 2;
            } else {
                NODAL_TRY(iteration((int)enqueued, c == 0));
                ++c;
                ++enqueued;
            }
        }
        double rr_now = -1.0;
        {
            const size_t bytes = (size_t)(2 * MAX_PARTIALS + F_COUNT) * 8;
            double *stage = poll_partials ? static_cast<double *>(nodal_pinned_arena(h, bytes)) : nullptr;
            if (stage) {
                NODAL_HIP_TRY(h, hipMemcpyAsync(stage, sb.part_rr, bytes, hipMemcpyDeviceToHost, st));
                NODAL_WAIT_STREAM(h, st);
                memcpy(hs, stage + 2 * MAX_PARTIALS, F_COUNT * 8);
                double acc = 0.0;
                for (int k = 0; k < sb.g0; ++k) acc += stage[k];
                rr_now = acc;
            } else {
                NODAL_TRY(nodal_read_words(h, hs, sb.sc, F_COUNT * 8));
            }
        }
        ++polls;
        bool conv = hs[F_CONV + ((enqueued - 1) & 1)] != 0.0;
        bool host_conv = false;
        if (!conv && rr_now >= 0.0 && hs[F_FLAG] == 0.0 && hs[F_BB] > 0.0 && rr_now <= tol * tol * hs[F_BB]) {
            host_conv = true;
            hs[F_RR] = rr_now;
            hs[F_ITERS] = (double)enqueued;
        } else if (!conv && rr_now >= 0.0) {
            hs[F_RR] = rr_now;
        }
        float ms = 0;
        if (!(conv && !host_conv && hs[F_ITERS] <= (double)(enqueued - batch)) && hipEventElapsedTime(&ms, e0, e1) == hipSuccess) {
            h->kern_ms += ms;
            h->kern_launches += 1;
        }
        if (hs[F_FLAG] != 0.0 || !(hs[F_RR] == hs[F_RR])) status = 2;
        else if (conv || host_conv) status = 1;
        else if (enqueued >= maxit) status = 3;
        else {
            int next = 2;
            const double target = tol * tol * hs[F_BB];
            const double rr_ref = rr_prev > 0.0 ? rr_prev : hs[F_BB];
            const int64_t it_ref = rr_prev > 0.0 ? it_prev : 0;
            if (hs[F_RR] > 0.0 && hs[F_RR] < rr_ref && enqueued > it_ref) {
                const double rate = log(hs[F_RR] / rr_ref) / (double)(enqueued - it_ref);
                static const double look = getenv("NODAL_FCG_LOOK") ? atof(getenv("NODAL_FCG_LOOK")) : 0.75;
                next = (int)floor(look * log(target / hs[F_RR]) / rate);
            }
            if (next > enqueued) next = (int)enqueued;
            batch = next < 1 ? 1 : (next > 32 ? 32 : next);
            rr_prev = hs[F_RR];
            it_prev = enqueued;
        }
    }
    const int64_t its = status == 1 ? (int64_t)hs[F_ITERS] : enqueued;
    *iters = (int32_t)its;
    *resid = hs[F_BB] > 0 ? sqrt(hs[F_RR] / hs[F_BB]) : 0.0;
    const SLevel *L0 = H->pool[0];
    h->kern_alg = 12.0 * (double)L0->nnz + 4.0 * (double)n + 16.0 * (double)n;
    if (fuse_dir) h->kern_alg += 12.0 * (double)n;
    if (trace)
        fprintf(stderr, "[sagg] %d iterations (%lld enqueued, %d polls), relative residual %.2e, status %d\n", *iters,
                (long long)enqueued, polls, *resid, status);
    if (trace && H->tail >= 0 && H->td.stamps) {
        long long ts[64];
        if (hipMemcpy(ts, H->td.stamps, sizeof ts, hipMemcpyDeviceToHost) == hipSuccess) {
            fprintf(stderr, "[sagg] tail phases (us):");
            for (int k = 1; k < (int)ts[63] && k < 63; ++k) fprintf(stderr, " %.2f", (double)(ts[k] - ts[k - 1]) * 0.01);
            fprintf(stderr, "  total %.2f, image %d B, lds %d B\n", (double)(ts[ts[63] - 1] - ts[0]) * 0.01,
                    H->td.image_bytes, H->td.lds_bytes);
            for (int k = 0; k < H->td.nlev; ++k)
                fprintf(stderr, "[sagg]   tail level %d: n %d width %d lpr %d nq %d\n", k, H->td.lv[k].n,
                        H->td.lv[k].width, H->td.lv[k].lpr, H->td.lv[k].nq);
        }
    }
    if (status != 1) {
        H->last_iters = 0;
        return -1;
    }
    H->last_iters = (int)its;
    H->hint_iters = (int)its;
    H->hint_n = n;
    H->hint_nnz = H->pool[0]->nnz;
    *info = 0;
    return NODAL_OK;
}

#include "sagg_multi.h"
```

Measured before the change: 147.3 circuits/s.

## Fuse small-level aggregation setup into a single-workgroup coarsen kernel

Refactors the per-level setup kernels (MIS, assign, build_P, restriction build/sort, AP rows) into device body functions and adds a single-block coarsen_small kernel. Once a level is small enough, it builds all remaining coarse levels, including the coarsest inverse, in one launch. This is meant to remove many tiny kernel launches and host round-trips in the setup of the deep, small levels. In exchange it runs serially on one workgroup with wave-level sync, adds a host readback of an outcome word, and makes the setup code much more complex.

```diff
diff --git a/nodal_amd/csrc/sagg.hip b/nodal_amd/csrc/sagg.hip
--- a/nodal_amd/csrc/sagg.hip
+++ b/nodal_amd/csrc/sagg.hip
@@ -39,13 +39,23 @@
     if (g >= 64) g = (g + 7) & ~(int64_t)7;
     return (unsigned)(g > cap ? cap : g);
 }
-inline int64_t pad64(int64_t n) { return (n + 63) & ~(int64_t)63; }
+__host__ __device__ inline int64_t pad64(int64_t n) { return (n + 63) & ~(int64_t)63; }
 
 __device__ __forceinline__ unsigned xcd_block() {
     const unsigned g = gridDim.x, b = blockIdx.x;
     return (g & 7u) ? b : (b & 7u) * (g >> 3) + (b >> 3);
 }
 
+template <bool WAVE>
+__device__ __forceinline__ void wave_sync() {
+    if constexpr (WAVE) {
+        __builtin_amdgcn_fence(__ATOMIC_RELEASE, "workgroup");
+        __builtin_amdgcn_wave_barrier();
+        __builtin_amdgcn_fence(__ATOMIC_ACQUIRE, "workgroup");
+    } else {
+        __syncthreads();
+    }
+}
 
 struct Ell {
     int64_t n = 0, ld = 0;
@@ -353,31 +363,18 @@
 }
 
 constexpr int64_t MIS_SMALL_MAX = 1024;
-__global__ __launch_bounds__(1024) void mis_small(Ell A, uint32_t *__restrict__ T, uint32_t *__restrict__ M,
-                                                  uint32_t *__restrict__ flag, int rounds) {
+__device__ __forceinline__ void mis_small_body(const Ell &A, uint32_t *__restrict__ T, uint32_t *__restrict__ M,
+                                               uint32_t *__restrict__ flag, int rounds) {
     const int64_t n = A.n;
     for (int64_t i = threadIdx.x; i < n; i += 1024) T[i] = (1u << 30) | hash30((uint32_t)i);
     __syncthreads();
     for (int r = 0; r < rounds; ++r) {
-        for (int64_t i = threadIdx.x; i < n; i += 1024) {
-            uint32_t best = T[i];
-            const int32_t l = A.len[i];
-            for (int32_t s = 0; s < l; ++s) {
-                const uint32_t t = T[A.col[(int64_t)s * A.ld + i]];
-                best = t > best ? t : best;
-            }
-            M[i] = best;
-        }
+        for (int64_t i = threadIdx.x; i < n; i += 1024) M[i] = nbr_max(A, T, i, A.len[i], T[i]);
         __syncthreads();
         for (int64_t i = threadIdx.x; i < n; i += 1024) {
             const uint32_t own = T[i];
             if ((own >> 30) != 1) continue;
-            uint32_t best = M[i];
-            const int32_t l = A.len[i];
-            for (int32_t s = 0; s < l; ++s) {
-                const uint32_t t = M[A.col[(int64_t)s * A.ld + i]];
-                best = t > best ? t : best;
-            }
+            const uint32_t best = nbr_max(A, M, i, A.len[i], M[i]);
             if (best == own) T[i] = own | (2u << 30);
             else if ((best >> 30) == 3) T[i] = 0;
         }
@@ -398,11 +395,14 @@
         flag[i] = f;
     }
 }
-
-__global__ __launch_bounds__(TB) void assign_near(Ell A, const uint32_t *__restrict__ T,
-                                                  const uint32_t *__restrict__ flag,
-                                                  const uint32_t *__restrict__ id, int32_t *__restrict__ agg1) {
-    for (int64_t i = (int64_t)xcd_block() * TB + threadIdx.x; i < A.n; i += (int64_t)gridDim.x * TB) {
+__global__ __launch_bounds__(1024) void mis_small(Ell A, uint32_t *__restrict__ T, uint32_t *__restrict__ M,
+                                                  uint32_t *__restrict__ flag, int rounds) {
+    mis_small_body(A, T, M, flag, rounds);
+}
+
+__device__ __forceinline__ void assign_near_body(const Ell &A, const uint32_t *__restrict__ T, const uint32_t *__restrict__ flag,
+                                                 const uint32_t *__restrict__ id, int32_t *__restrict__ agg1, unsigned vb, unsigned nb, unsigned tid) {
+    for (int64_t i = (int64_t)vb * TB + tid; i < A.n; i += (int64_t)nb * TB) {
         int32_t a = -1;
         if (flag[i]) a = (int32_t)id[i];
         else {
@@ -433,10 +433,15 @@
         agg1[i] = a;
     }
 }
-
-__global__ __launch_bounds__(TB) void assign_far(Ell A, const int32_t *__restrict__ agg1, int32_t *__restrict__ agg,
-                                                 unsigned long long *__restrict__ stats) {
-    for (int64_t i = (int64_t)xcd_block() * TB + threadIdx.x; i < A.n; i += (int64_t)gridDim.x * TB) {
+__global__ __launch_bounds__(TB) void assign_near(Ell A, const uint32_t *__restrict__ T,
+                                                  const uint32_t *__restrict__ flag,
+                                                  const uint32_t *__restrict__ id, int32_t *__restrict__ agg1) {
+    assign_near_body(A, T, flag, id, agg1, xcd_block(), gridDim.x, threadIdx.x);
+}
+
+__device__ __forceinline__ void assign_far_body(const Ell &A, const int32_t *__restrict__ agg1, int32_t *__restrict__ agg,
+                                                unsigned long long *__restrict__ stats, unsigned vb, unsigned nb, unsigned tid) {
+    for (int64_t i = (int64_t)vb * TB + tid; i < A.n; i += (int64_t)nb * TB) {
         int32_t a = agg1[i];
         if (a < 0) {
             double bw = -1.0;
@@ -467,11 +472,15 @@
         agg[i] = a;
     }
 }
-
-__global__ __launch_bounds__(TB) void build_P(Ell A, const double *__restrict__ dinv,
-                                              const int32_t *__restrict__ agg, int32_t *__restrict__ pcol,
-                                              double *__restrict__ pval, float *__restrict__ pvalf, double omega_p) {
-    for (int64_t i = (int64_t)xcd_block() * TB + threadIdx.x; i < A.n; i += (int64_t)gridDim.x * TB) {
+__global__ __launch_bounds__(TB) void assign_far(Ell A, const int32_t *__restrict__ agg1, int32_t *__restrict__ agg,
+                                                 unsigned long long *__restrict__ stats) {
+    assign_far_body(A, agg1, agg, stats, xcd_block(), gridDim.x, threadIdx.x);
+}
+
+__device__ __forceinline__ void build_P_body(const Ell &A, const double *__restrict__ dinv, const int32_t *__restrict__ agg,
+                                             int32_t *__restrict__ pcol, double *__restrict__ pval, float *__restrict__ pvalf,
+                                             double omega_p, unsigned vb, unsigned nb, unsigned tid) {
+    for (int64_t i = (int64_t)vb * TB + tid; i < A.n; i += (int64_t)nb * TB) {
         int32_t c[PW];
         double v[PW];
 #pragma unroll
@@ -503,10 +512,15 @@
         }
     }
 }
-
-__global__ __launch_bounds__(TB) void r_count(int64_t n, int64_t ld, const int32_t *__restrict__ pcol,
-                                              uint32_t *__restrict__ cnt, uint32_t *__restrict__ place) {
-    for (int64_t i = (int64_t)xcd_block() * TB + threadIdx.x; i < n; i += (int64_t)gridDim.x * TB) {
+__global__ __launch_bounds__(TB) void build_P(Ell A, const double *__restrict__ dinv,
+                                              const int32_t *__restrict__ agg, int32_t *__restrict__ pcol,
+                                              double *__restrict__ pval, float *__restrict__ pvalf, double omega_p) {
+    build_P_body(A, dinv, agg, pcol, pval, pvalf, omega_p, xcd_block(), gridDim.x, threadIdx.x);
+}
+
+__device__ __forceinline__ void r_count_body(int64_t n, int64_t ld, const int32_t *__restrict__ pcol, uint32_t *__restrict__ cnt,
+                                             uint32_t *__restrict__ place, unsigned vb, unsigned nb, unsigned tid) {
+    for (int64_t i = (int64_t)vb * TB + tid; i < n; i += (int64_t)nb * TB) {
 #pragma unroll
         for (int k = 0; k < PW; ++k) {
             const int32_t J = pcol[(int64_t)k * ld + i];
@@ -514,28 +528,36 @@
         }
     }
 }
+__global__ __launch_bounds__(TB) void r_count(int64_t n, int64_t ld, const int32_t *__restrict__ pcol,
+                                              uint32_t *__restrict__ cnt, uint32_t *__restrict__ place) {
+    r_count_body(n, ld, pcol, cnt, place, xcd_block(), gridDim.x, threadIdx.x);
+}
+__device__ __forceinline__ void r_fill_body(int64_t n, int64_t ld, const int32_t *__restrict__ pcol,
+                                            const uint32_t *__restrict__ rstart, const uint32_t *__restrict__ place,
+                                            uint64_t *__restrict__ keys, unsigned vb, unsigned nb, unsigned tid) {
+    for (int64_t i = (int64_t)vb * TB + tid; i < n; i += (int64_t)nb * TB) {
+#pragma unroll
+        for (int k = 0; k < PW; ++k) {
+            const int32_t J = pcol[(int64_t)k * ld + i];
+            if (J >= 0) keys[rstart[J] + place[(int64_t)k * ld + i]] = ((uint64_t)i << 2) | (uint64_t)k;
+        }
+    }
+}
 __global__ __launch_bounds__(TB) void r_fill(int64_t n, int64_t ld, const int32_t *__restrict__ pcol,
                                              const uint32_t *__restrict__ rstart, const uint32_t *__restrict__ place,
                                              uint64_t *__restrict__ keys) {
-    for (int64_t i = (int64_t)xcd_block() * TB + threadIdx.x; i < n; i += (int64_t)gridDim.x * TB) {
-#pragma unroll
-        for (int k = 0; k < PW; ++k) {
-            const int32_t J = pcol[(int64_t)k * ld + i];
-            if (J >= 0) keys[rstart[J] + place[(int64_t)k * ld + i]] = ((uint64_t)i << 2) | (uint64_t)k;
-        }
-    }
-}
-__global__ __launch_bounds__(TB) void r_to_ell(int64_t nc, int64_t rld, const uint32_t *__restrict__ rstart,
-                                               const uint64_t *__restrict__ keys, int64_t ld,
-                                               const double *__restrict__ pval, int32_t *__restrict__ rcol,
-                                               double *__restrict__ rval, float *__restrict__ rvalf,
-                                               int32_t *__restrict__ rlen,
-                                               unsigned long long *__restrict__ stats, uint32_t *__restrict__ bstat,
-                                               uint32_t rcap) {
+    r_fill_body(n, ld, pcol, rstart, place, keys, xcd_block(), gridDim.x, threadIdx.x);
+}
+__device__ __forceinline__ uint32_t r_to_ell_body(int64_t nc, int64_t rld, const uint32_t *__restrict__ rstart,
+                                                  const uint64_t *__restrict__ keys, int64_t ld,
+                                                  const double *__restrict__ pval, int32_t *__restrict__ rcol,
+                                                  double *__restrict__ rval, float *__restrict__ rvalf,
+                                                  int32_t *__restrict__ rlen, unsigned long long *__restrict__ stats,
+                                                  uint32_t rcap, unsigned vb, unsigned nb, unsigned tid) {
     uint32_t mlen = 0;
-    const int sub = threadIdx.x & 7;
-    const int64_t rows_per_pass = (int64_t)gridDim.x * (TB / 8);
-    for (int64_t I = (int64_t)xcd_block() * (TB / 8) + threadIdx.x / 8; I < nc; I += rows_per_pass) {
+    const int sub = tid & 7;
+    const int64_t rows_per_pass = (int64_t)nb * (TB / 8);
+    for (int64_t I = (int64_t)vb * (TB / 8) + tid / 8; I < nc; I += rows_per_pass) {
         const uint32_t s0 = rstart[I];
         uint32_t l = rstart[I + 1] - s0;
         mlen = l > mlen ? l : mlen;
@@ -559,6 +581,17 @@
         if (sub == 0) rlen[I] = (int32_t)l;
     }
     if (mlen > rcap) atomicOr(&stats[ST_OVERFLOW], 2ull);
+    return mlen;
+}
+__global__ __launch_bounds__(TB) void r_to_ell(int64_t nc, int64_t rld, const uint32_t *__restrict__ rstart,
+                                               const uint64_t *__restrict__ keys, int64_t ld,
+                                               const double *__restrict__ pval, int32_t *__restrict__ rcol,
+                                               double *__restrict__ rval, float *__restrict__ rvalf,
+                                               int32_t *__restrict__ rlen,
+                                               unsigned long long *__restrict__ stats, uint32_t *__restrict__ bstat,
+                                               uint32_t rcap) {
+    uint32_t mlen = r_to_ell_body(nc, rld, rstart, keys, ld, pval, rcol, rval, rvalf, rlen, stats, rcap, xcd_block(),
+                                  gridDim.x, threadIdx.x);
     __shared__ unsigned int s_max;
     if (threadIdx.x == 0) s_max = 0;
     __syncthreads();
@@ -598,29 +631,34 @@
     }
 }
 
-__global__ __launch_bounds__(TB) void r_sort_short(const uint32_t *__restrict__ rstart, uint64_t *__restrict__ keys,
-                                                   int64_t nc) {
-    for (int64_t I = (int64_t)xcd_block() * TB + threadIdx.x; I < nc; I += (int64_t)gridDim.x * TB) {
+template <int MAX_LEN = 32>
+__device__ __forceinline__ void r_sort_short_body(const uint32_t *__restrict__ rstart, uint64_t *__restrict__ keys,
+                                                  int64_t nc, unsigned vb, unsigned nb, unsigned tid) {
+    for (int64_t I = (int64_t)vb * TB + tid; I < nc; I += (int64_t)nb * TB) {
         const uint32_t s0 = rstart[I];
         const int len = (int)(rstart[I + 1] - s0);
         if (len < 2) continue;
         if (len <= 4) grp::sort_short_row<4>(keys + s0, len);
         else if (len <= 8) grp::sort_short_row<8>(keys + s0, len);
         else if (len <= 16) grp::sort_short_row<16>(keys + s0, len);
-        else if (len <= 32) grp::sort_short_row<32>(keys + s0, len);
-    }
-}
-__global__ __launch_bounds__(64) void r_sort_medium(const uint32_t *__restrict__ rstart, uint64_t *__restrict__ keys,
-                                                    int64_t nc) {
-    __shared__ uint64_t buf[RCAP_SMALL];
-    const int lane = threadIdx.x;
-    for (int64_t I = blockIdx.x; I < nc; I += gridDim.x) {
+        else if (len <= 32 && MAX_LEN >= 32) grp::sort_short_row<32>(keys + s0, len);
+    }
+}
+__global__ __launch_bounds__(TB) void r_sort_short(const uint32_t *__restrict__ rstart, uint64_t *__restrict__ keys,
+                                                   int64_t nc) {
+    r_sort_short_body(rstart, keys, nc, xcd_block(), gridDim.x, threadIdx.x);
+}
+template <bool WAVE, int MIN_LEN = 32>
+__device__ __forceinline__ void r_sort_medium_body(const uint32_t *__restrict__ rstart, uint64_t *__restrict__ keys,
+                                                   int64_t nc, int64_t I0, int64_t step, uint64_t *buf) {
+    const int lane = threadIdx.x & 63;
+    for (int64_t I = I0; I < nc; I += step) {
         const uint32_t s0 = rstart[I];
         const int len = (int)(rstart[I + 1] - s0);
-        if (len <= 32 || len > RCAP_SMALL) continue;
+        if (len <= MIN_LEN || len > RCAP_SMALL) continue;
         const int P = len <= 64 ? 64 : (len <= 128 ? 128 : (len <= 256 ? 256 : 512));
         for (int e = lane; e < P; e += 64) buf[e] = e < len ? keys[s0 + e] : ~0ull;
-        __syncthreads();
+        wave_sync<WAVE>();
         for (int size = 2; size <= P; size <<= 1)
             for (int stride = size >> 1; stride > 0; stride >>= 1) {
                 for (int p = lane; p < P / 2; p += 64) {
@@ -630,11 +668,16 @@
                     const uint64_t a = buf[i], b = buf[j];
                     if ((a > b) == up) { buf[i] = b; buf[j] = a; }
                 }
-                __syncthreads();
+                wave_sync<WAVE>();
             }
         for (int e = lane; e < len; e += 64) keys[s0 + e] = buf[e];
-        __syncthreads();
-    }
+        wave_sync<WAVE>();
+    }
+}
+__global__ __launch_bounds__(64) void r_sort_medium(const uint32_t *__restrict__ rstart, uint64_t *__restrict__ keys,
+                                                    int64_t nc) {
+    __shared__ uint64_t buf[RCAP_SMALL];
+    r_sort_medium_body<false>(rstart, keys, nc, blockIdx.x, gridDim.x, buf);
 }
 
 __device__ __forceinline__ int wave_excl_scan(int v, int *total) {
@@ -650,11 +693,13 @@
 }
 
 template <int APW>
-__global__ __launch_bounds__(TB) void ap_rows(Ell A, const int32_t *__restrict__ pcol, const double *__restrict__ pval,
-                                              int32_t *__restrict__ apcol, double *__restrict__ apval,
-                                              int32_t *__restrict__ aplen, unsigned long long *__restrict__ stats) {
+__device__ __forceinline__ void ap_rows_body(const Ell &A, const int32_t *__restrict__ pcol,
+                                             const double *__restrict__ pval, int32_t *__restrict__ apcol,
+                                             double *__restrict__ apval, int32_t *__restrict__ aplen,
+                                             unsigned long long *__restrict__ stats, unsigned vb, unsigned nb,
+                                             unsigned tid) {
     bool overflow = false;
-    for (int64_t i = (int64_t)xcd_block() * TB + threadIdx.x; i < A.n; i += (int64_t)gridDim.x * TB) {
+    for (int64_t i = (int64_t)vb * TB + tid; i < A.n; i += (int64_t)nb * TB) {
         int32_t c[APW];
         double v[APW];
 #pragma unroll
@@ -695,17 +740,22 @@
     }
     if (overflow) atomicOr(&stats[ST_OVERFLOW], 4ull);
 }
-
 template <int APW>
-__global__ __launch_bounds__(64) void ap_rows_lds(Ell A, const int32_t *__restrict__ pcol,
-                                                  const double *__restrict__ pval, int32_t *__restrict__ apcol,
-                                                  double *__restrict__ apval, int32_t *__restrict__ aplen,
-                                                  unsigned long long *__restrict__ stats) {
-    __shared__ int32_t tc[APW * 64];
-    __shared__ double tv[APW * 64];
-    const int lane = threadIdx.x;
+__global__ __launch_bounds__(TB) void ap_rows(Ell A, const int32_t *__restrict__ pcol, const double *__restrict__ pval,
+                                              int32_t *__restrict__ apcol, double *__restrict__ apval,
+                                              int32_t *__restrict__ aplen, unsigned long long *__restrict__ stats) {
+    ap_rows_body<APW>(A, pcol, pval, apcol, apval, aplen, stats, xcd_block(), gridDim.x, threadIdx.x);
+}
+
+template <int APW>
+__device__ __forceinline__ void ap_rows_lds_body(const Ell &A, const int32_t *__restrict__ pcol,
+                                                 const double *__restrict__ pval, int32_t *__restrict__ apcol,
+                                                 double *__restrict__ apval, int32_t *__restrict__ aplen,
+                                                 unsigned long long *__restrict__ stats, unsigned vb, unsigned nb,
+                                                 int32_t *tc, double *tv) {
+    const int lane = threadIdx.x & 63;
     bool overflow = false;
-    for (int64_t i0 = (int64_t)xcd_block() * 64; i0 < A.n; i0 += (int64_t)gridDim.x * 64) {
+    for (int64_t i0 = (int64_t)vb * 64; i0 < A.n; i0 += (int64_t)nb * 64) {
         const int64_t i = i0 + lane;
 #pragma unroll 8
         for (int q = 0; q < APW; ++q) tc[q * 64 + lane] = -1;
@@ -771,13 +821,23 @@
     }
     if (overflow) atomicOr(&stats[ST_OVERFLOW], 4ull);
 }
-
+template <int APW>
+__global__ __launch_bounds__(64) void ap_rows_lds(Ell A, const int32_t *__restrict__ pcol,
+                                                  const double *__restrict__ pval, int32_t *__restrict__ apcol,
+                                                  double *__restrict__ apval, int32_t *__restrict__ aplen,
+                                                  unsigned long long *__restrict__ stats) {
+    __shared__ int32_t tc[APW * 64];
+    __shared__ double tv[APW * 64];
+    ap_rows_lds_body<APW>(A, pcol, pval, apcol, apval, aplen, stats, xcd_block(), gridDim.x, tc, tv);
+}
+
+template <bool WAVE>
 __device__ __forceinline__ int galerkin_products(int64_t ld, const int32_t *__restrict__ apcol,
                                                  const double *__restrict__ apval, const int32_t *__restrict__ aplen,
                                                  int64_t rld, const int32_t *__restrict__ rcol,
                                                  const double *__restrict__ rval, int64_t I, int t0, int tn,
                                                  int32_t *lJ, double *lV) {
-    const int lane = threadIdx.x;
+    const int lane = threadIdx.x & 63;
     int32_t i = 0, len = 0;
     double w = 0.0;
     if (lane < tn) {
@@ -808,10 +868,134 @@
             }
     }
     for (int p = lane + np; p < np + 72; p += 64) lJ[p] = -1;
-    __syncthreads();
+    wave_sync<WAVE>();
     return np;
 }
 
+struct GalerkinSeen {
+    uint32_t max, nnz, flags;
+};
+template <bool NUMERIC, bool WAVE>
+__device__ __forceinline__ GalerkinSeen galerkin_body(int64_t ld, const int32_t *__restrict__ apcol,
+                                                      const double *__restrict__ apval, const int32_t *__restrict__ aplen,
+                                                      int64_t nc, int64_t rld, const int32_t *__restrict__ rcol,
+                                                      const double *__restrict__ rval, const int32_t *__restrict__ rlen,
+                                                      int64_t cld, int32_t *__restrict__ ccol, double *__restrict__ cval,
+                                                      float *__restrict__ cvalf, int32_t *__restrict__ clen,
+                                                      double *__restrict__ cdinv, int G, int pcap, int maxseg,
+                                                      int64_t I0, int64_t step, char *gsm) {
+    int32_t *set = reinterpret_cast<int32_t *>(gsm);
+    double *lV = reinterpret_cast<double *>(gsm + 1024);
+    int32_t *lJ = reinterpret_cast<int32_t *>(lV + pcap);
+    const int lane = threadIdx.x & 63;
+    uint32_t my_max = 0, my_nnz = 0, my_flags = 0;
+    for (int64_t I = I0; I < nc; I += step) {
+        const int rl = rlen[I];
+        const int ngroups = (rl + G - 1) / G;
+        int np = 0;
+        int total = 0;
+        int32_t myJ = 0x7fffffff;
+        if constexpr (NUMERIC) {
+            total = clen[I];
+            if (lane < total) myJ = ccol[(int64_t)lane * cld + I];
+        } else {
+        for (int k = lane; k < 256; k += 64) set[k] = -1;
+        wave_sync<WAVE>();
+        for (int g = 0; g < ngroups; ++g) {
+            np = galerkin_products<WAVE>(ld, apcol, apval, aplen, rld, rcol, rval, I, g * G, min(G, rl - g * G), lJ, lV);
+            for (int p = lane; p < np; p += 64) {
+                const int32_t J = lJ[p];
+                uint32_t hsh = ((uint32_t)J * 2654435761u) >> 24;
+                for (int probe = 0; probe < 256; ++probe) {
+                    const int32_t old = atomicCAS(&set[hsh], -1, J);
+                    if (old == -1 || old == J) break;
+                    hsh = (hsh + 1) & 255u;
+                    if (probe == 255) my_flags |= 1u;
+                }
+            }
+            wave_sync<WAVE>();
+        }
+        int32_t mine[4];
+        int cnt = 0;
+#pragma unroll
+        for (int q = 0; q < 4; ++q) {
+            mine[q] = set[lane * 4 + q];
+            cnt += mine[q] >= 0 ? 1 : 0;
+        }
+        int off = wave_excl_scan(cnt, &total);
+        wave_sync<WAVE>();
+#pragma unroll
+        for (int q = 0; q < 4; ++q)
+            if (mine[q] >= 0) set[off++] = mine[q];
+        wave_sync<WAVE>();
+        if (total > ACAP) {
+            my_flags |= 1u;
+            total = ACAP;
+        }
+        myJ = lane < total ? set[lane] : 0x7fffffff;
+        wave_sync<WAVE>();
+#pragma unroll
+        for (int k = 2; k <= 64; k <<= 1) {
+#pragma unroll
+            for (int j = k >> 1; j > 0; j >>= 1) {
+                const int32_t other = __shfl_xor(myJ, j, 64);
+                const bool up = (lane & k) == 0, lower = (lane & j) == 0;
+                const int32_t lo = myJ < other ? myJ : other, hi = myJ < other ? other : myJ;
+                myJ = (lower == up) ? lo : hi;
+            }
+        }
+        }
+        const int nseg = min(maxseg, total <= 16 ? 4 : (total <= 32 ? 2 : 1)), segw = 64 / nseg;
+        const int seg = lane / segw;
+        const int32_t segJ = __shfl(myJ, lane % segw, 64);
+        double acc = 0.0;
+        for (int g = 0; g < ngroups; ++g) {
+            if (ngroups > 1 || NUMERIC)
+                np = galerkin_products<WAVE>(ld, apcol, apval, aplen, rld, rcol, rval, I, g * G, min(G, rl - g * G), lJ, lV);
+            int chunk = (((np + nseg - 1) / nseg) + 7) & ~7;
+            if (nseg > 1 && ((chunk >> 3) & 1) == 0) chunk += 8;
+            for (int p = seg * chunk; p < (seg + 1) * chunk; p += 8) {
+                int32_t j8[8];
+                double v8[8];
+#pragma unroll
+                for (int u = 0; u < 8; ++u) {
+                    j8[u] = lJ[p + u];
+                    v8[u] = lV[p + u];
+                }
+#pragma unroll
+                for (int u = 0; u < 8; ++u) acc += j8[u] == segJ ? v8[u] : 0.0;
+            }
+            wave_sync<WAVE>();
+        }
+        if (nseg == 4) {
+            const double a1 = __shfl(acc, lane + 16, 64), a2 = __shfl(acc, lane + 32, 64), a3 = __shfl(acc, lane + 48, 64);
+            acc = (acc + a1) + (a2 + a3);
+        } else if (nseg == 2) {
+            acc += __shfl(acc, lane + 32, 64);
+        }
+        if (lane >= total && lane < APAD) {
+            ccol[(int64_t)lane * cld + I] = (int32_t)I;
+            cval[(int64_t)lane * cld + I] = 0.0;
+            cvalf[(int64_t)lane * cld + I] = 0.0f;
+        }
+        if (lane < total) {
+            ccol[(int64_t)lane * cld + I] = myJ;
+            cval[(int64_t)lane * cld + I] = acc;
+            cvalf[(int64_t)lane * cld + I] = (float)acc;
+            if (myJ == (int32_t)I) {
+                if (!(acc > 0.0)) my_flags |= 4u;
+                cdinv[I] = acc > 0.0 ? 1.0 / acc : 1.0;
+            }
+        }
+        if (lane == 0) {
+            clen[I] = total;
+            my_max = (uint32_t)total > my_max ? (uint32_t)total : my_max;
+            my_nnz += (uint32_t)total;
+        }
+        wave_sync<WAVE>();
+    }
+    return GalerkinSeen{my_max, my_nnz, my_flags};
+}
 template <bool NUMERIC>
 __global__ __launch_bounds__(64) void galerkin(int64_t ld, const int32_t *__restrict__ apcol,
                                                const double *__restrict__ apval, const int32_t *__restrict__ aplen,
@@ -823,156 +1007,54 @@
                                                unsigned long long *__restrict__ stats, uint32_t *__restrict__ bstat,
                                                int G, int pcap, int maxseg) {
     extern __shared__ __attribute__((aligned(16))) char gsm[];
-    int32_t *set = reinterpret_cast<int32_t *>(gsm);
-    double *lV = reinterpret_cast<double *>(gsm + 1024);
-    int32_t *lJ = reinterpret_cast<int32_t *>(lV + pcap);
-    const int lane = threadIdx.x;
-    uint32_t my_max = 0, my_nnz = 0, my_flags = 0;
-    for (int64_t I = blockIdx.x; I < nc; I += gridDim.x) {
-        const int rl = rlen[I];
-        const int ngroups = (rl + G - 1) / G;
-        int np = 0;
-        int total = 0;
-        int32_t myJ = 0x7fffffff;
-        if constexpr (NUMERIC) {
-            total = clen[I];
-            if (lane < total) myJ = ccol[(int64_t)lane * cld + I];
-        } else {
-        for (int k = lane; k < 256; k += 64) set[k] = -1;
-        __syncthreads();
-        for (int g = 0; g < ngroups; ++g) {
-            np = galerkin_products(ld, apcol, apval, aplen, rld, rcol, rval, I, g * G, min(G, rl - g * G), lJ, lV);
-            for (int p = lane; p < np; p += 64) {
-                const int32_t J = lJ[p];
-                uint32_t hsh = ((uint32_t)J * 2654435761u) >> 24;
-                for (int probe = 0; probe < 256; ++probe) {
-                    const int32_t old = atomicCAS(&set[hsh], -1, J);
-                    if (old == -1 || old == J) break;
-                    hsh = (hsh + 1) & 255u;
-                    if (probe == 255) my_flags |= 1u;
-                }
-            }
-            __syncthreads();
-        }
-        int32_t mine[4];
-        int cnt = 0;
-#pragma unroll
-        for (int q = 0; q < 4; ++q) {
-            mine[q] = set[lane * 4 + q];
-            cnt += mine[q] >= 0 ? 1 : 0;
-        }
-        int off = wave_excl_scan(cnt, &total);
-        __syncthreads();
-#pragma unroll
-        for (int q = 0; q < 4; ++q)
-            if (mine[q] >= 0) set[off++] = mine[q];
-        __syncthreads();
-        if (total > ACAP) {
-            my_flags |= 1u;
-            total = ACAP;
-        }
-        myJ = lane < total ? set[lane] : 0x7fffffff;
-        __syncthreads();
-#pragma unroll
-        for (int k = 2; k <= 64; k <<= 1) {
-#pragma unroll
-            for (int j = k >> 1; j > 0; j >>= 1) {
-                const int32_t other = __shfl_xor(myJ, j, 64);
-                const bool up = (lane & k) == 0, lower = (lane & j) == 0;
-                const int32_t lo = myJ < other ? myJ : other, hi = myJ < other ? other : myJ;
-                myJ = (lower == up) ? lo : hi;
-            }
-        }
-        }
-        const int nseg = min(maxseg, total <= 16 ? 4 : (total <= 32 ? 2 : 1)), segw = 64 / nseg;
-        const int seg = lane / segw;
-        const int32_t segJ = __shfl(myJ, lane % segw, 64);
-        double acc = 0.0;
-        for (int g = 0; g < ngroups; ++g) {
-            if (ngroups > 1 || NUMERIC)
-                np = galerkin_products(ld, apcol, apval, aplen, rld, rcol, rval, I, g * G, min(G, rl - g * G), lJ, lV);
-            int chunk = (((np + nseg - 1) / nseg) + 7) & ~7;
-            if (nseg > 1 && ((chunk >> 3) & 1) == 0) chunk += 8;
-            for (int p = seg * chunk; p < (seg + 1) * chunk; p += 8) {
-                int32_t j8[8];
-                double v8[8];
-#pragma unroll
-                for (int u = 0; u < 8; ++u) {
-                    j8[u] = lJ[p + u];
-                    v8[u] = lV[p + u];
-                }
-#pragma unroll
-                for (int u = 0; u < 8; ++u) acc += j8[u] == segJ ? v8[u] : 0.0;
-            }
-            __syncthreads();
-        }
-        if (nseg == 4) {
-            const double a1 = __shfl(acc, lane + 16, 64), a2 = __shfl(acc, lane + 32, 64), a3 = __shfl(acc, lane + 48, 64);
-            acc = (acc + a1) + (a2 + a3);
-        } else if (nseg == 2) {
-            acc += __shfl(acc, lane + 32, 64);
-        }
-        if (lane >= total && lane < APAD) {
-            ccol[(int64_t)lane * cld + I] = (int32_t)I;
-            cval[(int64_t)lane * cld + I] = 0.0;
-            cvalf[(int64_t)lane * cld + I] = 0.0f;
-        }
-        if (lane < total) {
-            ccol[(int64_t)lane * cld + I] = myJ;
-            cval[(int64_t)lane * cld + I] = acc;
-            cvalf[(int64_t)lane * cld + I] = (float)acc;
-            if (myJ == (int32_t)I) {
-                if (!(acc > 0.0)) my_flags |= 4u;
-                cdinv[I] = acc > 0.0 ? 1.0 / acc : 1.0;
-            }
-        }
-        if (lane == 0) {
-            clen[I] = total;
-            my_max = (uint32_t)total > my_max ? (uint32_t)total : my_max;
-            my_nnz += (uint32_t)total;
-        }
-        __syncthreads();
-    }
-    if (lane == 0) {
-        bstat[blockIdx.x] = my_max;
-        bstat[BSTAT_MAX + blockIdx.x] = my_nnz;
-    }
-    if (my_flags & 1u) atomicOr(&stats[ST_OVERFLOW], 1ull);
-    if (my_flags & 4u) atomicOr(&stats[ST_BADDIAG], 1ull);
-}
-
-__global__ __launch_bounds__(256) void coarsest_inverse(Ell A, double *__restrict__ inv,
-                                                        unsigned long long *__restrict__ stats) {
-    __shared__ double M[COARSEST][2 * COARSEST + 1];
+    const GalerkinSeen seen = galerkin_body<NUMERIC, false>(ld, apcol, apval, aplen, nc, rld, rcol, rval, rlen, cld, ccol,
+                                                            cval, cvalf, clen, cdinv, G, pcap, maxseg, blockIdx.x,
+                                                            gridDim.x, gsm);
+    if (threadIdx.x == 0) {
+        bstat[blockIdx.x] = seen.max;
+        bstat[BSTAT_MAX + blockIdx.x] = seen.nnz;
+    }
+    if (seen.flags & 1u) atomicOr(&stats[ST_OVERFLOW], 1ull);
+    if (seen.flags & 4u) atomicOr(&stats[ST_BADDIAG], 1ull);
+}
+
+__device__ __forceinline__ void coarsest_inverse_body(const Ell &A, double *__restrict__ inv,
+                                                      unsigned long long *__restrict__ stats, int tid, int nt,
+                                                      double (*M)[2 * COARSEST + 1]) {
     const int n = (int)A.n;
-    for (int t = threadIdx.x; t < n * 2 * n; t += 256) {
+    for (int t = tid; t < n * 2 * n; t += nt) {
         const int r = t / (2 * n), c = t % (2 * n);
         M[r][c] = (c >= n && c - n == r) ? 1.0 : 0.0;
     }
     __syncthreads();
-    for (int r = threadIdx.x; r < n; r += 256)
+    for (int r = tid; r < n; r += nt)
         for (int s = 0; s < A.len[r]; ++s) M[r][A.col[(int64_t)s * A.ld + r]] = A.val[(int64_t)s * A.ld + r];
     __syncthreads();
     for (int k = 0; k < n; ++k) {
         const double pv = M[k][k];
         if (!(pv > 0.0)) {
-            if (threadIdx.x == 0) atomicOr(&stats[ST_BADDIAG], 2ull);
+            if (tid == 0) atomicOr(&stats[ST_BADDIAG], 2ull);
             return;
         }
         const double rp = 1.0 / pv;
         __syncthreads();
-        for (int c = threadIdx.x; c < 2 * n; c += 256) M[k][c] *= rp;
+        for (int c = tid; c < 2 * n; c += nt) M[k][c] *= rp;
         __syncthreads();
-        for (int t = threadIdx.x; t < n * 2 * n; t += 256) {
+        for (int t = tid; t < n * 2 * n; t += nt) {
             const int r = t / (2 * n), c = t % (2 * n);
             if (r != k && c != k) M[r][c] = fma(-M[r][k], M[k][c], M[r][c]);
         }
         __syncthreads();
-        for (int r = threadIdx.x; r < n; r += 256)
+        for (int r = tid; r < n; r += nt)
             if (r != k) M[r][k] = 0.0;
         __syncthreads();
     }
-    for (int t = threadIdx.x; t < n * n; t += 256) inv[t] = M[t / n][n + t % n];
+    for (int t = tid; t < n * n; t += nt) inv[t] = M[t / n][n + t % n];
+}
+__global__ __launch_bounds__(256) void coarsest_inverse(Ell A, double *__restrict__ inv,
+                                                        unsigned long long *__restrict__ stats) {
+    __shared__ double M[COARSEST][2 * COARSEST + 1];
+    coarsest_inverse_body(A, inv, stats, threadIdx.x, 256, M);
 }
 
 __global__ __launch_bounds__(TB) void flags_up(int64_t n, const int32_t *__restrict__ agg,
@@ -1019,6 +1101,198 @@
         if (!grounded[i]) *floating = 1;
 }
 
+constexpr int64_t SMALL_SETUP_MAX = 1024;
+constexpr int SMALL_THREADS = 1024;
+constexpr int SMALL_LEVELS = 4;
+constexpr int SMALL_AP_WAVES = 3;
+constexpr int SMALL_LDS = SMALL_AP_WAVES * 64 * 64 * 12;
+static_assert(SMALL_LDS >= COARSEST * (2 * COARSEST + 1) * 8, "coarsest inverse");
+static_assert(SMALL_LDS >= (SMALL_THREADS / 64) * RCAP_SMALL * 8, "medium sorts");
+enum { FX_OUTCOME = 0, FX_LEVEL = 1, FX_INV = 2, FX_WORDS = 8 };
+enum { FX_BREAK = 1 , FX_STOP = 2 , FX_DECLINED = 3,
+       FX_RESUME = 4 , FX_MAXLEV = 5 };
+
+__host__ __device__ inline int galerkin_group(int apw, int g_env) {
+    int G = 1024 / apw;
+    G = (G < 8 ? 8 : (G > 64 ? 64 : G));
+    if (g_env >= 8 && g_env <= 64 && apw == 16) G = g_env & ~7;
+    return G;
+}
+
+struct SmallLevel {
+    int32_t *acol, *alen, *agg, *pcol, *rcol, *rlen;
+    double *aval, *dinv, *pval, *rval;
+    float *avalf, *pvalf, *rvalf;
+};
+struct SmallArgs {
+    int l0, nlev_max;
+    int64_t n0, ld0;
+    int32_t maxlen0;
+    SmallLevel lv[SMALL_LEVELS + 1];
+    uint32_t *T, *M, *flag, *id, *rstart, *place;
+    int32_t *agg1, *apcol, *aplen;
+    uint64_t *keys;
+    double *apval, *inv;
+    unsigned long long *stats;
+    double omega0, omega1;
+    int mis_rounds, g_env, maxseg;
+    long long *stamps;
+};
+
+__device__ __forceinline__ void small_phase_sync() { __syncthreads(); }
+__device__ __forceinline__ void small_stamp(long long *stamps, int &at) {
+    if (stamps && threadIdx.x == 0 && at < 256) stamps[at] = (long long)__builtin_amdgcn_s_memrealtime();
+    ++at;
+}
+
+__device__ __forceinline__ uint32_t small_scan(const uint32_t *in, uint32_t *out, int64_t len, uint32_t *part) {
+    const int lane = threadIdx.x & 63, wave = threadIdx.x >> 6;
+    uint32_t carry = 0;
+    for (int64_t base = 0; base < len; base += SMALL_THREADS) {
+        const int64_t i = base + threadIdx.x;
+        const uint32_t v = i < len ? in[i] : 0u;
+        uint32_t incl = v;
+#pragma unroll
+        for (int off = 1; off < 64; off <<= 1) {
+            const uint32_t t = __shfl_up(incl, off, 64);
+            if (lane >= off) incl += t;
+        }
+        if (lane == 63) part[wave] = incl;
+        __syncthreads();
+        uint32_t before = 0, tot = 0;
+#pragma unroll
+        for (int w = 0; w < SMALL_THREADS / 64; ++w) {
+            const uint32_t s = part[w];
+            if (w < wave) before += s;
+            tot += s;
+        }
+        if (i < len) out[i] = carry + before + incl - v;
+        carry += tot;
+        __syncthreads();
+    }
+    return carry;
+}
+
+__global__ __launch_bounds__(SMALL_THREADS) void coarsen_small(SmallArgs a) {
+    extern __shared__ __attribute__((aligned(16))) char sm[];
+    __shared__ uint32_t s_part[SMALL_THREADS / 64];
+    __shared__ uint32_t s_rmax, s_gmax;
+    __shared__ unsigned long long s_gnnz;
+    const unsigned t = threadIdx.x, vb = t / TB, nb = SMALL_THREADS / TB, tid = t % TB;
+    const int wave = (int)(t >> 6), lane = (int)(t & 63);
+    unsigned long long *fx = a.stats + (size_t)MAX_LEVELS * ST_COUNT;
+    int64_t n = a.n0, ld = a.ld0;
+    int l = a.l0, k = 0, outcome, at = 0;
+    small_stamp(a.stamps, at);
+    for (;; ++l, ++k) {
+        if (n <= COARSEST && l > 0) { outcome = FX_BREAK; break; }
+        if (l + 1 >= MAX_LEVELS) { outcome = FX_MAXLEV; break; }
+        if (k >= a.nlev_max) { outcome = FX_RESUME; break; }
+        const SmallLevel &L = a.lv[k], &C = a.lv[k + 1];
+        Ell A;
+        A.n = n; A.ld = ld; A.col = L.acol; A.val = L.aval; A.len = L.alen;
+        unsigned long long *st = a.stats + (size_t)l * ST_COUNT, *cst = st + ST_COUNT;
+        mis_small_body(A, a.T, a.M, a.flag, a.mis_rounds);
+        small_phase_sync();
+        small_stamp(a.stamps, at);
+        const uint32_t nc32 = small_scan(a.flag, a.id, n + 1, s_part);
+        if (t == 0) *reinterpret_cast<uint32_t *>(st + ST_NC) = nc32;
+        small_phase_sync();
+        small_stamp(a.stamps, at);
+        assign_near_body(A, a.T, a.flag, a.id, a.agg1, vb, nb, tid);
+        small_phase_sync();
+        small_stamp(a.stamps, at);
+        assign_far_body(A, a.agg1, L.agg, st, vb, nb, tid);
+        small_phase_sync();
+        small_stamp(a.stamps, at);
+        build_P_body(A, L.dinv, L.agg, L.pcol, L.pval, L.pvalf, l > 0 ? a.omega1 : a.omega0, vb, nb, tid);
+        small_phase_sync();
+        small_stamp(a.stamps, at);
+        const int64_t nc = nc32;
+        int32_t maxlen = a.maxlen0;
+        if (l > 0) {
+            maxlen = (int32_t)st[ST_MAXLEN];
+            const unsigned long long *up = st - ST_COUNT;
+            if (st[ST_OVERFLOW] || st[ST_BADDIAG] || up[ST_OVERFLOW] || up[ST_UNASSIGNED]) { outcome = FX_DECLINED; break; }
+        }
+        if (nc >= n || maxlen <= 1) { outcome = FX_STOP; break; }
+        if ((nc * 2 > n && n > 4096) || nc < 1) { outcome = FX_DECLINED; break; }
+        const int64_t cld = pad64(nc);
+        const uint32_t rcap = nc <= RCAP_SMALL_ROWS ? RCAP_SMALL : RCAP;
+        for (int64_t i = t; i <= nc; i += SMALL_THREADS) a.rstart[i] = 0;
+        small_phase_sync();
+        small_stamp(a.stamps, at);
+        r_count_body(n, ld, L.pcol, a.rstart, a.place, vb, nb, tid);
+        small_phase_sync();
+        small_stamp(a.stamps, at);
+        (void)small_scan(a.rstart, a.rstart, nc + 1, s_part);
+        small_phase_sync();
+        small_stamp(a.stamps, at);
+        r_fill_body(n, ld, L.pcol, a.rstart, a.place, a.keys, vb, nb, tid);
+        small_phase_sync();
+        small_stamp(a.stamps, at);
+        r_sort_short_body<16>(a.rstart, a.keys, nc, vb, nb, tid);
+        r_sort_medium_body<true, 16>(a.rstart, a.keys, nc, wave, SMALL_THREADS / 64,
+                                     reinterpret_cast<uint64_t *>(sm) + (size_t)wave * RCAP_SMALL);
+        if (t == 0) { s_rmax = 0; s_gmax = 0; s_gnnz = 0; }
+        small_phase_sync();
+        small_stamp(a.stamps, at);
+        const uint32_t rl = r_to_ell_body(nc, cld, a.rstart, a.keys, ld, L.pval, L.rcol, L.rval, L.rvalf, L.rlen, st, rcap,
+                                          vb, nb, tid);
+        atomicMax(&s_rmax, rl);
+        const int apw = maxlen <= 6 ? 16 : 64;
+        if (apw == 16) {
+            ap_rows_body<16>(A, L.pcol, L.pval, a.apcol, a.apval, a.aplen, st, vb, nb, tid);
+        } else if (wave < SMALL_AP_WAVES) {
+            char *slice = sm + (size_t)wave * 64 * 64 * 12;
+            ap_rows_lds_body<64>(A, L.pcol, L.pval, a.apcol, a.apval, a.aplen, st, wave, SMALL_AP_WAVES,
+                                 reinterpret_cast<int32_t *>(slice), reinterpret_cast<double *>(slice + 64 * 64 * 4));
+        }
+        small_phase_sync();
+        small_stamp(a.stamps, at);
+        if (t == 0) st[ST_MAXR] = s_rmax;
+        const int G = galerkin_group(apw, a.g_env), pcap = G * apw + 72;
+        const int slice = (1024 + pcap * 12 + 15) & ~15;
+        const int gw = SMALL_LDS / slice < SMALL_THREADS / 64 ? SMALL_LDS / slice : SMALL_THREADS / 64;
+        if (wave < gw) {
+            const GalerkinSeen seen = galerkin_body<false, true>(ld, a.apcol, a.apval, a.aplen, nc, cld, L.rcol, L.rval,
+                                                                 L.rlen, cld, C.acol, C.aval, C.avalf, C.alen, C.dinv,
+                                                                 G, pcap, a.maxseg, wave, gw, sm + (size_t)wave * slice);
+            if (lane == 0) {
+                atomicMax(&s_gmax, seen.max);
+                atomicAdd(&s_gnnz, (unsigned long long)seen.nnz);
+            }
+            if (seen.flags & 1u) atomicOr(&cst[ST_OVERFLOW], 1ull);
+            if (seen.flags & 4u) atomicOr(&cst[ST_BADDIAG], 1ull);
+        }
+        small_phase_sync();
+        small_stamp(a.stamps, at);
+        if (t == 0) {
+            cst[ST_MAXLEN] = s_gmax;
+            cst[ST_NNZ] = s_gnnz;
+        }
+        small_phase_sync();
+        small_stamp(a.stamps, at);
+        n = nc;
+        ld = cld;
+    }
+    small_stamp(a.stamps, at);
+    if (t == 0) {
+        fx[FX_OUTCOME] = (unsigned long long)outcome;
+        fx[FX_LEVEL] = (unsigned long long)l;
+    }
+    if ((outcome == FX_BREAK || outcome == FX_STOP) && l > 0 && a.stats[(size_t)l * ST_COUNT + ST_MAXLEN] > 1 &&
+        n <= COARSEST) {
+        Ell A;
+        A.n = n; A.ld = ld; A.col = a.lv[k].acol; A.val = a.lv[k].aval; A.len = a.lv[k].alen;
+        if (t == 0) fx[FX_INV] = 1;
+        coarsest_inverse_body(A, a.inv, a.stats + (size_t)l * ST_COUNT, (int)t, SMALL_THREADS,
+                              reinterpret_cast<double(*)[2 * COARSEST + 1]>(sm));
+    }
+    __syncthreads();
+    small_stamp(a.stamps, at);
+}
+
 }
 
 #include "sagg_cycle.h"
@@ -1051,6 +1325,20 @@
     cyc_t *z, *x0;
     int g0;
 };
+
+int sa_gg() {
+    static const int g_env = getenv("NODAL_SA_GG") ? atoi(getenv("NODAL_SA_GG")) : 40;
+    return g_env;
+}
+int sa_gseg() {
+    static const int maxseg = getenv("NODAL_SA_GSEG") ? atoi(getenv("NODAL_SA_GSEG")) : 4;
+    return maxseg;
+}
+int sa_mis_rounds() {
+    static const int mis_rounds =
+        getenv("NODAL_SA_MIS") ? std::min(MIS_ROUNDS, std::max(1, atoi(getenv("NODAL_SA_MIS")))) : MIS_ROUNDS;
+    return mis_rounds;
+}
 
 template <bool NUMERIC>
 int galerkin_product(nodal_ctx *h, SHierarchy *H, int l, hipEvent_t r_ready = nullptr, int phase = 0) {
@@ -1079,14 +1367,11 @@
         NODAL_HIP_TRY(h, hipGetLastError());
     }
     if (phase == 1) return NODAL_OK;
-    int G = 1024 / apw;
-    G = (G < 8 ? 8 : (G > 64 ? 64 : G));
-    static const int g_env = getenv("NODAL_SA_GG") ? atoi(getenv("NODAL_SA_GG")) : 40;
-    if (g_env >= 8 && g_env <= 64 && apw == 16) G = g_env & ~7;
+    const int G = galerkin_group(apw, sa_gg());
     const int pcap = G * apw + 72;
     const size_t lds = 1024 + (size_t)pcap * 12;
     static const int64_t gcap = getenv("NODAL_SA_GCAP") ? atoll(getenv("NODAL_SA_GCAP")) : 16384;
-    static const int maxseg = getenv("NODAL_SA_GSEG") ? atoi(getenv("NODAL_SA_GSEG")) : 4;
+    const int maxseg = sa_gseg();
     const unsigned gg = (unsigned)(nc < gcap ? nc : (gcap < BSTAT_MAX ? gcap : BSTAT_MAX));
     if (r_ready) NODAL_HIP_TRY(h, hipStreamWaitEvent(st, r_ready, 0));
     galerkin<NUMERIC><<<gg, 64, lds, st>>>(
@@ -1138,7 +1423,7 @@
     const unsigned g = grid_for(n);
     static const bool trace_mis = getenv("NODAL_TRACE") != nullptr;
     if (trace_mis) NODAL_HIP_TRY(h, hipMemsetAsync(cnt, 0, (MIS_ROUNDS + 2) * 8, st));
-    static const int mis_rounds = getenv("NODAL_SA_MIS") ? std::min(MIS_ROUNDS, std::max(1, atoi(getenv("NODAL_SA_MIS")))) : MIS_ROUNDS;
+    const int mis_rounds = sa_mis_rounds();
     if (n <= MIS_SMALL_MAX && !trace_mis) {
         mis_small<<<1, 1024, 0, st>>>(A, T, M, flag, mis_rounds);
     } else {
@@ -1297,6 +1582,123 @@
     return NODAL_OK;
 }
 
+int coarsen_small_run(nodal_ctx *h, SHierarchy *H, int l0, unsigned long long *hs, int *outcome, int *lend, bool *inv) {
+    hipStream_t st = h->stream;
+    unsigned long long *dstats = H->stats.as<unsigned long long>();
+    const int64_t n = H->level(l0)->n, ldb = H->level(l0)->ld;
+    const int nlev_max = std::min(SMALL_LEVELS, MAX_LEVELS - 1 - l0);
+    const size_t a4 = (((size_t)(n + 1) * 4) + 255) & ~(size_t)255;
+    NODAL_HIP_TRY(h, H->mis_t.reserve((size_t)n * 8 + 64));
+    NODAL_HIP_TRY(h, H->mis_m.reserve((size_t)n * 8 + 64));
+    NODAL_HIP_TRY(h, H->mis_flag.reserve((size_t)(n + 1) * 4 + 64));
+    NODAL_HIP_TRY(h, H->mis_id.reserve((size_t)(n + 1) * 4 + 64));
+    NODAL_HIP_TRY(h, H->agg1.reserve((size_t)n * 4 + 64));
+    NODAL_HIP_TRY(h, H->rstart.reserve(a4 + (size_t)PW * ldb * 4 + 64));
+    NODAL_HIP_TRY(h, H->keys.reserve((size_t)PW * n * 8 + 64));
+    NODAL_HIP_TRY(h, H->apcol.reserve((size_t)64 * ldb * 4 + 64));
+    NODAL_HIP_TRY(h, H->apval.reserve((size_t)64 * ldb * 8 + 64));
+    NODAL_HIP_TRY(h, H->aplen.reserve((size_t)ldb * 4 + 64));
+    NODAL_HIP_TRY(h, H->coarse_inv.reserve((size_t)COARSEST * COARSEST * 8 + 64));
+    for (int k = 0; k <= nlev_max; ++k) {
+        SLevel *L = H->level(l0 + k);
+        if (k > 0) {
+            NODAL_HIP_TRY(h, L->acol.reserve((size_t)ACAP * ldb * 4 + 64));
+            NODAL_HIP_TRY(h, L->aval.reserve((size_t)ACAP * ldb * 8 + 64));
+            NODAL_HIP_TRY(h, L->avalf.reserve((size_t)ACAP * ldb * 4 + 64));
+            NODAL_HIP_TRY(h, L->alen.reserve((size_t)ldb * 4 + 64));
+            NODAL_HIP_TRY(h, L->dinv.reserve((size_t)ldb * 8 + 64));
+        }
+        if (k == nlev_max) break;
+        NODAL_HIP_TRY(h, L->agg.reserve((size_t)n * 4 + 64));
+        NODAL_HIP_TRY(h, L->pcol.reserve((size_t)PW * ldb * 4 + 64));
+        NODAL_HIP_TRY(h, L->pval.reserve((size_t)PW * ldb * 8 + 64));
+        NODAL_HIP_TRY(h, L->pvalf.reserve((size_t)PW * ldb * 4 + 64));
+        NODAL_HIP_TRY(h, L->rcol.reserve((size_t)RCAP_SMALL * ldb * 4 + 64));
+        NODAL_HIP_TRY(h, L->rval.reserve((size_t)RCAP_SMALL * ldb * 8 + 64));
+        NODAL_HIP_TRY(h, L->rvalf.reserve((size_t)RCAP_SMALL * ldb * 4 + 64));
+        NODAL_HIP_TRY(h, L->rlen.reserve((size_t)ldb * 4 + 64));
+    }
+    SmallArgs a;
+    memset(&a, 0, sizeof a);
+    a.l0 = l0;
+    a.nlev_max = nlev_max;
+    a.n0 = n;
+    a.ld0 = ldb;
+    a.maxlen0 = H->level(l0)->maxlen;
+    for (int k = 0; k <= nlev_max; ++k) {
+        const SLevel *L = H->pool[l0 + k];
+        SmallLevel &q = a.lv[k];
+        q.acol = L->acol.as<int32_t>(); q.alen = L->alen.as<int32_t>(); q.aval = L->aval.as<double>();
+        q.avalf = L->avalf.as<float>(); q.dinv = L->dinv.as<double>();
+        q.agg = L->agg.as<int32_t>(); q.pcol = L->pcol.as<int32_t>(); q.pval = L->pval.as<double>();
+        q.pvalf = L->pvalf.as<float>(); q.rcol = L->rcol.as<int32_t>(); q.rval = L->rval.as<double>();
+        q.rvalf = L->rvalf.as<float>(); q.rlen = L->rlen.as<int32_t>();
+    }
+    a.T = H->mis_t.as<uint32_t>(); a.M = H->mis_m.as<uint32_t>();
+    a.flag = H->mis_flag.as<uint32_t>(); a.id = H->mis_id.as<uint32_t>();
+    a.rstart = H->rstart.as<uint32_t>(); a.place = reinterpret_cast<uint32_t *>(H->rstart.as<char>() + a4);
+    a.agg1 = H->agg1.as<int32_t>();
+    a.apcol = H->apcol.as<int32_t>(); a.aplen = H->aplen.as<int32_t>(); a.apval = H->apval.as<double>();
+    a.keys = H->keys.as<uint64_t>();
+    a.inv = H->coarse_inv.as<double>();
+    a.stats = dstats;
+    a.omega0 = omega_p(0);
+    a.omega1 = omega_p(1);
+    a.mis_rounds = sa_mis_rounds();
+    a.g_env = sa_gg();
+    a.maxseg = sa_gseg();
+    static const bool probe = getenv("NODAL_SA_SMALL_PROBE") != nullptr;
+    if (probe) {
+        NODAL_HIP_TRY(h, H->tail_stamps.reserve(256 * sizeof(long long)));
+        NODAL_HIP_TRY(h, hipMemsetAsync(H->tail_stamps.p, 0, 256 * sizeof(long long), st));
+        a.stamps = H->tail_stamps.as<long long>();
+    }
+    {
+        static std::atomic<bool> lds_allowed[64];
+        const int dev = h->device >= 0 && h->device < 64 ? h->device : 0;
+        if (!lds_allowed[dev].load(std::memory_order_acquire)) {
+            NODAL_HIP_TRY(h, hipFuncSetAttribute(reinterpret_cast<const void *>(coarsen_small),
+                                                 hipFuncAttributeMaxDynamicSharedMemorySize, SMALL_LDS));
+            lds_allowed[dev].store(true, std::memory_order_release);
+        }
+    }
+    coarsen_small<<<1, SMALL_THREADS, SMALL_LDS, st>>>(a);
+    NODAL_HIP_TRY(h, hipGetLastError());
+    NODAL_HIP_TRY(h, hipMemcpyAsync(hs, dstats, (size_t)(MAX_LEVELS * ST_COUNT + FX_WORDS) * 8, hipMemcpyDeviceToHost, st));
+    if (!H->ev_copy) NODAL_HIP_TRY(h, hipEventCreateWithFlags(&H->ev_copy, hipEventDisableTiming));
+    NODAL_HIP_TRY(h, hipEventRecord(H->ev_copy, st));
+    NODAL_WAIT_EVENT(h, H->ev_copy, st);
+    const unsigned long long *fx = hs + (size_t)MAX_LEVELS * ST_COUNT;
+    *outcome = (int)fx[FX_OUTCOME];
+    *lend = (int)fx[FX_LEVEL];
+    *inv = fx[FX_INV] != 0;
+    if (probe) {
+        long long ts[256];
+        NODAL_HIP_TRY(h, hipMemcpy(ts, H->tail_stamps.p, sizeof ts, hipMemcpyDeviceToHost));
+        fprintf(stderr, "[sagg] coarsen_small levels %d..%d, phases (us):", l0, *lend);
+        for (int i = 1; i < 256 && ts[i]; ++i) fprintf(stderr, " %.1f", (ts[i] - ts[i - 1]) / 100.0);
+        fprintf(stderr, "\n");
+    }
+    if (*outcome < FX_BREAK || *outcome > FX_MAXLEV || *lend < l0 || *lend > l0 + nlev_max) {
+        return nodal_fail(h, NODAL_E_HIP, "sagg: coarsen_small left no verdict");
+    }
+    for (int l = l0; l < *lend; ++l) {
+        SLevel *L = H->pool[l], *C = H->pool[l + 1];
+        const int64_t nc = (int64_t)(hs[(size_t)l * ST_COUNT + ST_NC] & 0xffffffffull);
+        L->nc = nc;
+        C->n = nc;
+        C->ld = pad64(nc);
+        C->width = ACAP;
+        C->nc = 0;
+        L->rld = C->ld;
+        if (l > 0) {
+            L->maxlen = (int32_t)hs[(size_t)l * ST_COUNT + ST_MAXLEN];
+            L->nnz = (int64_t)hs[(size_t)l * ST_COUNT + ST_NNZ];
+        }
+    }
+    return NODAL_OK;
+}
+
 const void *tail_kernel(int slots) {
     return slots <= 8 ? reinterpret_cast<const void *>(k_tail<8>)
                       : slots <= 16 ? reinterpret_cast<const void *>(k_tail<16>)
@@ -1493,12 +1895,13 @@
     H->flags_levels = 0;
     H->last_iters = 0;
     H->drop_graph();
-    NODAL_HIP_TRY(h, H->stats.reserve((size_t)MAX_LEVELS * ST_COUNT * 8 + 64));
+    NODAL_HIP_TRY(h, H->stats.reserve((size_t)(MAX_LEVELS * ST_COUNT + FX_WORDS) * 8 + 64));
     if (!H->host_stats)
-        NODAL_HIP_TRY(h, hipHostMalloc(reinterpret_cast<void **>(&H->host_stats), (size_t)MAX_LEVELS * ST_COUNT * 8 + 64));
+        NODAL_HIP_TRY(h, hipHostMalloc(reinterpret_cast<void **>(&H->host_stats),
+                                       (size_t)(MAX_LEVELS * ST_COUNT + FX_WORDS) * 8 + 64));
     unsigned long long *dstats = H->stats.as<unsigned long long>();
     unsigned long long *hs = reinterpret_cast<unsigned long long *>(H->host_stats);
-    NODAL_HIP_TRY(h, hipMemsetAsync(dstats, 0, (size_t)MAX_LEVELS * ST_COUNT * 8, st));
+    NODAL_HIP_TRY(h, hipMemsetAsync(dstats, 0, (size_t)(MAX_LEVELS * ST_COUNT + FX_WORDS) * 8, st));
     NODAL_HIP_TRY(h, H->bstat.reserve((size_t)2 * BSTAT_MAX * 4 + 64));
     {
         const unsigned gr = grid_for(n0);
@@ -1541,6 +1944,10 @@
 
     int l = 0;
     bool diag_last = false;
+    static const bool fused = !(getenv("NODAL_SA_FUSED_SETUP") && atoi(getenv("NODAL_SA_FUSED_SETUP")) == 0) &&
+                              getenv("NODAL_TRACE") == nullptr;
+    bool stats_fresh = false;
+    bool inv_done = false;
     for (;; ++l) {
         SLevel *L = H->level(l);
         if (L->n <= COARSEST && l > 0) break;
@@ -1549,7 +1956,27 @@
             return NODAL_OK;
         }
         bool declined = false, stop = false;
-        NODAL_TRY(build_level(h, H, l, hs, &declined, &stop));
+        if (fused && L->n <= SMALL_SETUP_MAX) {
+            int outcome = 0, lend = l;
+            NODAL_TRY(coarsen_small_run(h, H, l, hs, &outcome, &lend, &inv_done));
+            stats_fresh = true;
+            l = lend;
+            L = H->level(l);
+            if (outcome == FX_RESUME) {
+                --l;
+                continue;
+            }
+            if (outcome == FX_BREAK) break;
+            if (outcome == FX_MAXLEV) {
+                if (trace) fprintf(stderr, "[sagg] declined: more than %d levels\n", MAX_LEVELS);
+                return NODAL_OK;
+            }
+            stop = outcome == FX_STOP;
+            declined = outcome == FX_DECLINED;
+        } else {
+            stats_fresh = false;
+            NODAL_TRY(build_level(h, H, l, hs, &declined, &stop));
+        }
         if (declined) {
             if (trace)
                 fprintf(stderr, "[sagg] declined at level %d (%lld rows): does not coarsen / over a cap / not positive "
@@ -1568,9 +1995,11 @@
     H->nlev = l + 1;
     SLevel *last = H->level(l);
     if (H->nlev < 2) return NODAL_OK;
-    NODAL_HIP_TRY(h, hipMemcpyAsync(hs, dstats, (size_t)MAX_LEVELS * ST_COUNT * 8, hipMemcpyDeviceToHost, st));
-    if (!H->ev_copy) NODAL_HIP_TRY(h, hipEventCreateWithFlags(&H->ev_copy, hipEventDisableTiming));
-    NODAL_HIP_TRY(h, hipEventRecord(H->ev_copy, st));
+    if (!stats_fresh) {
+        NODAL_HIP_TRY(h, hipMemcpyAsync(hs, dstats, (size_t)MAX_LEVELS * ST_COUNT * 8, hipMemcpyDeviceToHost, st));
+        if (!H->ev_copy) NODAL_HIP_TRY(h, hipEventCreateWithFlags(&H->ev_copy, hipEventDisableTiming));
+        NODAL_HIP_TRY(h, hipEventRecord(H->ev_copy, st));
+    }
     if (check_floating) {
         if (H->flags_levels == 0) {
             NODAL_HIP_TRY(h, H->level(0)->gflag.reserve((size_t)n0 + 64));
@@ -1606,9 +2035,11 @@
     if (H->dense_coarsest) {
         if (last->n > COARSEST) return NODAL_OK;
         NODAL_HIP_TRY(h, H->coarse_inv.reserve((size_t)last->n * last->n * 8 + 64));
-        coarsest_inverse<<<1, 256, 0, st>>>(last->A(), H->coarse_inv.as<double>(),
-                                            dstats + (size_t)l * ST_COUNT);
-        NODAL_HIP_TRY(h, hipGetLastError());
+        if (!(stats_fresh && inv_done)) {
+            coarsest_inverse<<<1, 256, 0, st>>>(last->A(), H->coarse_inv.as<double>(),
+                                                dstats + (size_t)l * ST_COUNT);
+            NODAL_HIP_TRY(h, hipGetLastError());
+        }
     }
     for (int k = 0; k < H->nlev; ++k) {
         SLevel *L = H->pool[k];
```

After: 148.2 circuits/s, median of 6. No clear change (+0.6%).
